# real-stanford/garmentnets

Hardware: AMD Instinct MI355X
Metric: garments/s end-to-end predict (PointNet++ -> gridding -> UNet3D -> WNF decode -> marching cubes) (higher is better)
Workload: dtype f32 (f16x2 convs, f16x2 decoder MLPs, fp32 accumulation)

## Files before the change

garmentnets_amd/_lib.py:

```python
import ctypes
import os

_HERE = os.path.dirname(os.path.abspath(__file__))
LIB_PATH = os.environ.get("GARMENTNETS_HIP_LIB") or os.path.join(_HERE, "libgarmentnets_hip.so")

GN_OK, GN_EINVAL, GN_ELAUNCH, GN_ECAP = 0, -1, -2, -3

_vp, _i32, _i64, _f32, _f64, _sz = (ctypes.c_void_p, ctypes.c_int, ctypes.c_int64, ctypes.c_float, ctypes.c_double,
                                   ctypes.c_size_t)

PROTOTYPES = {
    "gn_version": [],
    "gn_device_info": [_vp, _vp],
    "gn_segment_ptr": [_vp, _i64, _i32, _vp, _vp],
    "gn_fps": [_vp, _vp, _vp, _vp, _i32, _i32, _vp, _vp],
    "gn_fps_nested": [_vp, _vp, _vp, _vp, _i32, _i32, _vp, _vp, _vp, _vp],
    "gn_fps_workspace_bytes": [_i32, _i32],
    "gn_fps_nested_ws": [_vp, _vp, _vp, _vp, _i32, _i32, _vp, _vp, _vp, _vp, _sz, _vp],
    "gn_ball_query": [_vp, _vp, _vp, _vp, _i32, _i32, _f32, _i32, _vp, _vp, _vp],
    "gn_sa_gather": [_vp, _i32, _i32, _vp, _vp, _vp, _i32, _i32, _i32, _vp, _i32, _vp, _vp],
    "gn_segment_max": [_vp, _i32, _vp, _i32, _i32, _i32, _vp, _i32, _vp],
    "gn_sa_fused_supported": [_i32, _i32, _i32, _i32],
    "gn_sa_fused": [_vp, _i32, _i32, _vp, _vp, _vp, _vp, _i32, _i32, _i32, _vp, _vp, _vp, _vp, _i32, _i32, _i32, _vp, _i32, _vp],
    "gn_sa_fused_scoped": [_vp, _i32, _i32, _vp, _vp, _vp, _vp, _i32, _i32, _i32, _vp, _vp, _vp, _vp, _vp, _i32, _i32, _i32, _vp, _i32, _vp],
    "gn_sa_fused_group": [_vp, _i32, _i32, _vp, _vp, _vp, _vp, _i32, _i32, _i32, _vp, _vp, _vp, _vp, _vp, _i32, _i32, _i32, _vp, _i32, _vp, _i32],
    "gn_sa_fused_auto_group": [_i32, _i32, _i32, _i32, _i32],
    "gn_sa_gather_scoped": [_vp, _i32, _i32, _vp, _vp, _vp, _i32, _i32, _i32, _vp, _vp, _i32, _vp, _vp],
    "gn_global_max_pool": [_vp, _i32, _vp, _i32, _i32, _vp, _i32, _vp],
    "gn_knn_interpolate": [_vp, _i32, _vp, _vp, _vp, _vp, _i32, _i32, _i32, _i32, _vp, _i32, _vp],
    "gn_knn_interpolate_any": [_vp, _i32, _vp, _vp, _vp, _vp, _i32, _i32, _i32, _i32, _vp, _i32, _vp],
    "gn_linear": [_vp, _i32, _vp, _i32, _vp, _vp, _vp, _i32, _i64, _i32, _i32, _vp, _i32, _vp],
    "gn_nocs_head": [_vp, _i32, _i64, _i32, _vp, _vp, _vp, _vp],
    "gn_grid_features": [_vp, _i32, _i32, _vp, _vp, _vp, _vp, _i64, _vp, _vp, _vp, _i32, _i32, _vp, _i32, _vp, _vp],
    "gn_grid_scatter_workspace_bytes": [_i64, _i32, _i32],
    "gn_grid_scatter": [_vp, _i32, _vp, _i64, _i32, _i64, _i32, _vp, _vp, _vp, _sz, _i32, _vp],
    "gn_grid_scatter_ex": [_vp, _i32, _vp, _i64, _i32, _i32, _i64, _i32, _vp, _vp, _vp, _sz, _i32, _vp],
    "gn_channel_stats": [_vp, _i32, _i64, _i32, _vp, _vp, _vp],
    "gn_groupnorm_affine": [_vp, _vp, _i32, _i64, _vp, _vp, _i32, _i64, _i32, _i32, _i32, _f32, _vp, _vp, _vp, _vp, _vp, _vp],
    "gn_channel_stats_any": [_vp, _i32, _i64, _i32, _vp, _vp, _vp],
    "gn_groupnorm_affine_map": [_vp, _vp, _i32, _i32, _i64, _vp, _vp, _i32, _i32, _i64, _i32, _i32, _i32, _f32, _vp, _vp, _vp, _vp, _vp, _vp],
    "gn_conv3d_gcr": [_vp, _i32, _vp, _i32, _vp, _vp, _vp, _i32, _i32, _i32, _i32, _i32, _i32, _vp, _vp, _vp, _vp],
    "gn_conv3d_gcr_split": [_vp, _i32, _vp, _i32, _vp, _vp, _vp, _i32, _vp, _vp, _i32, _i32, _i32, _i32, _i32, _i32, _vp, _vp, _vp, _vp, _vp, _i32, _vp, _vp, _sz, _vp],
    "gn_conv3d_occupancy_workspace_bytes": [_i32, _i32, _i32, _i32],
    "gn_conv_affine_pack_bytes": [_i32, _i32, _i32],
    "gn_conv_affine_pack": [_vp, _i32, _i32, _vp, _vp, _vp, _vp, _i64, _vp, _i32, _vp, _sz, _vp, _vp, _vp, _vp, _vp, _sz, _vp],
    "gn_conv3d_gcr_split_persample": [_vp, _i32, _vp, _vp, _vp, _vp, _vp, _i32, _i32, _i32, _i32, _i32, _i32, _vp, _vp, _vp, _vp, _vp, _i32, _vp, _vp, _sz, _vp],
    "gn_conv_affine_pack_wino_bytes": [_i32, _i32, _i32],
    "gn_conv_affine_pack_wino": [_vp, _i32, _i32, _vp, _vp, _vp, _vp, _i64, _vp, _i32, _vp, _sz, _vp, _vp, _vp, _vp, _vp, _sz, _vp],
    "gn_conv3d_gcr_split_wino": [_vp, _i32, _vp, _vp, _vp, _vp, _vp, _vp, _i32, _i32, _i32, _i32, _i32, _i32, _vp, _vp, _vp, _vp, _vp, _i32, _vp, _sz, _vp],
    "gn_conv3d_gcr_split_wino_partial": [_vp, _i32, _vp, _vp, _vp, _vp, _vp, _vp, _i32, _i32, _i32, _i32, _i32, _i32, _vp, _vp, _vp, _vp, _vp],
    "gn_weight_pack_split_bytes": [_i32, _i32, _i32],
    "gn_weight_pack_split_wino_bytes": [_i32, _i32],
    "gn_weight_pack_upconv_bytes": [_i32, _i32],
    "gn_weight_pack_split": [_vp, _i32, _i32, _i32, _i32, _i32, _vp, _sz, _vp, _vp],
    "gn_weight_pack_split_wino": [_vp, _i32, _i32, _i32, _i32, _vp, _sz, _vp, _vp],
    "gn_weight_pack_upconv": [_vp, _i32, _i32, _i32, _i32, _vp, _sz, _vp, _vp],
    "gn_affine_act": [_vp, _i32, _i64, _i32, _vp, _vp, _vp, _i32, _vp, _vp],
    "gn_upconv_partial": [_vp, _i32, _vp, _vp, _vp, _i32, _vp, _vp, _i32, _i32, _i32, _i32, _i32, _vp, _vp],
    "gn_grid_tile_flags": [_vp, _i64, _i32, _i32, _i32, _i32, _i32, _vp, _vp],
    "gn_maxpool3d_2": [_vp, _i32, _i32, _i32, _i32, _i32, _vp, _vp, _vp, _vp],
    "gn_grid_stats": [_vp, _vp, _i64, _i32, _i64, _i32, _vp, _vp, _vp, _vp],
    "gn_trilinear_sample": [_vp, _i32, _i32, _i32, _i32, _vp, _i32, _i64, _i64, _vp, _i32, _vp],
    "gn_trilinear_sample_batch": [_vp, _i32, _i64, _i32, _i32, _i32, _i32, _vp, _i64, _vp, _i32, _vp],
    "gn_implicit_decode": [_vp, _i32, _i32, _i32, _i32, _vp, _i32, _vp, _i32, _i64, _i64, _vp, _vp, _vp, _vp, _i32, _vp, _vp, _vp, _vp, _i32,
                           _vp, _vp, _vp, _vp, _i32, _vp, _i32, _vp, _vp],
    "gn_ggm3d": [_vp, _i32, _i32, _i32, _f64, _vp, _vp, _vp],
    "gn_minmax": [_vp, _i64, _vp, _vp],
    "gn_ggm3d_batch": [_vp, _i32, _i32, _i32, _i32, _f64, _vp, _vp, _vp],
    "gn_ggm3d_range_workspace_bytes": [_i32, _i32, _i32, _i32],
    "gn_ggm3d_batch_ex": [_vp, _i32, _i32, _i32, _i32, _f64, _vp, _vp, _i32, _vp, _vp, _sz, _vp],
    "gn_minmax_batch": [_vp, _i32, _i64, _vp, _vp],
    "gn_mc33_batch_workspace_bytes": [_i32, _i32, _i32, _i32],
    "gn_mc33_batch": [_vp, _i32, _i32, _i32, _i32, _f64, _vp, _sz, _vp, _vp, _vp, _vp, _i64, _i64, _vp, _vp],
    "gn_mc33_batch_profiled": [_vp, _i32, _i32, _i32, _i32, _f64, _vp, _sz, _vp, _vp, _vp, _vp, _i64, _i64, _vp, _vp, _vp],
    "gn_mc33_workspace_bytes": [_i32, _i32, _i32],
    "gn_mc33": [_vp, _i32, _i32, _i32, _f64, _vp, _sz, _vp, _vp, _vp, _vp, _i64, _i64, _vp, _vp],
    "gn_gather_nn": [_vp, _i32, _i32, _i32, _vp, _i64, _f64, _vp, _vp],
    "gn_gather_nn_batch": [_vp, _i32, _i32, _i32, _i32, _vp, _i64, _f64, _vp, _vp],
    "gn_mesh_compact_workspace_bytes": [_i64, _i64],
    "gn_mesh_largest_component_workspace_bytes": [_i64],
    "gn_mesh_largest_component": [_vp, _i64, _i64, _vp, _sz, _vp, _vp, _vp, _vp],
    "gn_mesh_compact": [_vp, _i32, _vp, _vp, _i64, _i64, _vp, _sz, _vp, _vp, _vp, _vp],
    "gn_scale_verts": [_vp, _i64, _f64, _vp, _vp],
    "gn_implicit_decode_split": [_vp, _i32, _i64, _vp, _vp, _vp, _i32, _i32, _i32, _i32, _vp, _i32, _vp],
    "gn_implicit_decode_split_batch": [_vp, _i32, _i64, _i32, _vp, _vp, _vp, _i32, _i32, _i32, _i32, _vp, _i32, _vp],
    "gn_implicit_decode_batch": [_vp, _i32, _i64, _i32, _i32, _vp, _vp, _vp, _vp, _i32, _vp, _vp, _vp, _vp, _i32, _vp, _vp, _vp, _vp, _i32, _vp, _i32, _vp, _i32, _vp],
    "gn_implicit_decode_lattice_split": [_vp, _i32, _i32, _i32, _i32, _i32, _i64, _i64, _vp, _vp, _vp, _i32, _i32, _i32, _vp, _i32, _vp],
    "gn_decoder_input_scale": [_vp, _i64, _i32, _i32, _f32, _vp, _vp],
    "gn_nearest_neighbor": [_vp, _i64, _vp, _i64, _vp, _vp, _vp],
    "gn_nearest_neighbor_f64_batch": [_vp, _vp, _vp, _i32, _i64, _vp, _vp, _vp],
    "gn_point_mesh_sqdist_batch": [_vp, _vp, _vp, _vp, _i32, _i64, _vp, _vp, _vp, _vp],
    "gn_winding_number_batch": [_vp, _vp, _vp, _vp, _i32, _i64, _vp, _vp, _vp],
    "gn_winding_field_batch": [_vp, _vp, _vp, _i32, _i32, _i32, _i32, _vp, _vp, _vp],
    "gn_distance_field_batch": [_vp, _vp, _vp, _i32, _i32, _i32, _i32, _vp, _vp, _vp, _vp],
    "gn_query_targets_face_chunk": [],
    "gn_query_targets_workspace_bytes": [_i32, _i64, _i64, _i32],
    "gn_query_targets_batch": [_vp, _vp, _vp, _vp, _i32, _i64, _i64, _i32, _i32, _f32, _i32, _vp, _sz, _vp, _vp, _vp, _vp, _vp, _vp],
    "gn_nocs_bin_metrics_workspace_bytes": [_vp, _i32],
    "gn_nocs_bin_metrics": [_vp, _i32, _i32, _i32, _vp, _sz, _vp, _vp],
    "gn_value_losses_workspace_bytes": [_vp, _i32],
    "gn_value_losses": [_vp, _i32, _vp, _sz, _vp, _vp],
    "gn_nocs_bin_loss_bwd": [_vp, _i32, _i32, _i32, _vp, _vp, _vp, _vp],
    "gn_value_losses_bwd": [_vp, _i32, _vp, _vp, _vp],
    "gn_adam_step": [_vp, _i32, _i64, _vp, _i32, _vp],
    "gn_grad_pack": [_vp, _i32, _i64, _vp, _i64, _i32, _vp],
    "gn_grid_scatter_bwd_workspace_bytes": [_i64, _i32, _i64, _i32],
    "gn_grid_scatter_bwd": [_vp, _vp, _vp, _i32, _vp, _i64, _i32, _i32, _i64, _i32, _vp, _sz, _vp, _i32, _vp],
    "gn_segment_max_bwd": [_vp, _i32, _vp, _i32, _vp, _i32, _vp, _i32, _i32, _i32, _vp, _i32, _vp],
    "gn_global_max_pool_bwd": [_vp, _i32, _vp, _i32, _vp, _i32, _vp, _i32, _i32, _vp, _i32, _vp],
    "gn_sa_gather_bwd_workspace_bytes": [_i64, _i64],
    "gn_sa_gather_bwd": [_vp, _i32, _vp, _i64, _i32, _i64, _vp, _sz, _vp, _i32, _vp],
    "gn_knn_neighbours": [_vp, _vp, _vp, _vp, _i32, _i32, _i32, _vp, _vp, _vp],
    "gn_knn_interpolate_bwd_workspace_bytes": [_i64, _i32, _i64],
    "gn_knn_interpolate_bwd": [_vp, _vp, _i32, _i32, _vp, _i32, _i32, _i32, _vp, _sz, _vp, _i32, _vp],
    "gn_trilinear_sample_bwd_workspace_bytes": [_i32, _i64, _i32, _i32, _i32],
    "gn_trilinear_sample_bwd": [_vp, _i32, _vp, _i32, _i32, _i32, _i32, _i32, _vp, _i64, _vp, _sz, _vp, _vp, _vp],
    "gn_conv3d_bwd_weight_workspace_bytes": [_i32, _i32, _i32, _i32, _i32, _i32],
    "gn_conv3d_bwd_weight": [_vp, _i32, _vp, _i32, _vp, _vp, _vp, _vp, _i32, _i32, _i32, _i32, _i32, _vp, _sz, _vp, _vp],
    "gn_relu_mask": [_vp, _vp, _i64, _vp, _vp],
    "gn_relu_mask_max_workspace_bytes": [_i32],
    "gn_relu_mask_max": [_vp, _vp, _i32, _i64, _i32, _vp, _vp, _vp, _vp, _vp, _sz, _vp],
    "gn_conv3d_bwd_weight_split_workspace_bytes": [_i32, _i32, _i32, _i32, _i32, _i32],
    "gn_conv3d_bwd_weight_split": [_vp, _i32, _vp, _i32, _vp, _vp, _vp, _vp, _vp, _vp, _i32, _i32, _i32, _i32, _i32, _vp, _sz, _vp, _vp],
    "gn_groupnorm_bwd_stats_workspace_bytes": [_i32, _i64, _i32],
    "gn_groupnorm_bwd_stats": [_vp, _i32, _i32, _vp, _i32, _i32, _i32, _i32, _i32, _i32, _vp, _sz, _vp, _vp, _vp],
    "gn_groupnorm_bwd_coef": [_vp, _vp, _vp, _vp, _i32, _i32, _i64, _vp, _vp, _vp, _vp, _i32, _i32, _i64, _i32, _i32, _i32, _f32, _vp, _vp, _vp, _vp, _vp,
                              _vp, _vp],
    "gn_groupnorm_bwd_apply": [_vp, _i32, _i32, _vp, _i32, _i32, _i32, _i32, _i32, _i32, _vp, _vp, _vp, _i32, _i32, _i32, _vp, _vp],
    "gn_maxpool3d_2_bwd": [_vp, _vp, _i32, _i32, _i32, _i32, _i32, _vp, _vp],
    "gn_linear_act_bwd_workspace_bytes": [_i64, _i32],
    "gn_linear_act_bwd": [_vp, _i32, _vp, _i32, _vp, _i64, _i32, _vp, _i32, _vp, _sz, _vp, _vp],
    "gn_linear_bwd_weight_workspace_bytes": [_i64, _i32, _i32],
    "gn_linear_bwd_weight": [_vp, _i32, _vp, _i32, _i64, _i32, _i32, _vp, _sz, _vp, _i32, _vp],
    "gn_row_affine": [_vp, _i32, _vp, _vp, _i64, _i32, _vp, _i32, _vp],
    "gn_col_moments_workspace_bytes": [_i64, _i32],
    "gn_col_moments": [_vp, _i32, _i64, _i32, _vp, _sz, _vp, _vp],
    "gn_col_dots_workspace_bytes": [_i64, _i32],
    "gn_col_dots": [_vp, _i32, _vp, _i32, _i64, _i32, _vp, _sz, _vp, _vp],
    "gn_bn_train_bwd_workspace_bytes": [_i64, _i32],
    "gn_bn_train_bwd": [_vp, _i32, _vp, _i32, _vp, _i64, _i32, _vp, _i32, _vp, _sz, _vp, _vp],
    "gn_resident_points": [_vp, _vp, _i32, _i32, _vp, _vp, _vp, _vp, _vp, _vp, _vp, _vp],
    "gn_resident_garment": [_vp, _vp, _i32, _i32, _vp, _vp, _vp, _vp, _vp, _vp, _vp, _vp, _vp, _vp],
    "gn_resident_volume": [_vp, _vp, _i32, _i32, _i32, _vp, _vp, _vp, _vp, _vp, _i32, _vp, _vp, _vp],
    "gn_resident_volume_queries": [_vp, _vp, _i32, _i32, _i32, _vp, _vp, _vp, _vp, _vp, _vp, _vp, _vp],
    "gn_resident_query_targets": [_vp, _vp, _i32, _i64, _i32, _i64, _i64, _i32, _i32, _f32, _i32, _vp, _vp, _sz, _vp, _vp, _vp],
    "gn_resident_surface": [_vp, _vp, _i32, _i32, _vp, _vp, _i32, _vp, _vp, _vp, _vp],
    "gn_resident_mc_surface": [_vp, _vp, _i32, _i32, _vp, _vp, _vp, _vp, _vp],
    "gn_render_points_batch": [_vp, _vp, _vp, _vp, _vp, _i32, _i32, _vp, _vp],
    "gn_color_idx_batch": [_vp, _vp, _vp, _vp, _vp, _i32, _i32, _vp, _vp],
}
_RESTYPES = {"gn_weight_pack_split_bytes": _sz, "gn_weight_pack_split_wino_bytes": _sz, "gn_weight_pack_upconv_bytes": _sz,
             "gn_conv_affine_pack_bytes": _sz, "gn_conv_affine_pack_wino_bytes": _sz, "gn_conv3d_occupancy_workspace_bytes": _sz, "gn_mc33_workspace_bytes": _sz, "gn_ggm3d_range_workspace_bytes": _sz, "gn_mc33_batch_workspace_bytes": _sz, "gn_grid_scatter_workspace_bytes": _sz, "gn_fps_workspace_bytes": _sz, "gn_mesh_compact_workspace_bytes": _sz, "gn_mesh_largest_component_workspace_bytes": _sz,
             "gn_nocs_bin_metrics_workspace_bytes": _sz, "gn_value_losses_workspace_bytes": _sz,
             "gn_grid_scatter_bwd_workspace_bytes": _sz, "gn_sa_gather_bwd_workspace_bytes": _sz, "gn_knn_interpolate_bwd_workspace_bytes": _sz,
             "gn_trilinear_sample_bwd_workspace_bytes": _sz, "gn_conv3d_bwd_weight_workspace_bytes": _sz, "gn_conv3d_bwd_weight_split_workspace_bytes": _sz, "gn_relu_mask_max_workspace_bytes": _sz, "gn_groupnorm_bwd_stats_workspace_bytes": _sz,
             "gn_linear_act_bwd_workspace_bytes": _sz, "gn_linear_bwd_weight_workspace_bytes": _sz,
             "gn_col_moments_workspace_bytes": _sz, "gn_col_dots_workspace_bytes": _sz, "gn_bn_train_bwd_workspace_bytes": _sz,
             "gn_query_targets_workspace_bytes": _sz}

LINEAR_BWD_CHUNK_ROWS = 512
LINEAR_ACT_CHUNK_ROWS = 1024

LOSS_MAX_SETS = 8
LOSS_KINDS = {"l2": 0, "smooth_l1": 1, "bce_logits": 2, "row_norm": 3}


class NocsBinSet(ctypes.Structure):
    _fields_ = [("logits", _vp), ("gt", _vp), ("n", _i64), ("ldl", _i32), ("pad", _i32)]


class LossSegment(ctypes.Structure):
    _fields_ = [("pred", _vp), ("target", _vp), ("count", _i64), ("kind", _i32), ("mirror", _i32)]


class NocsBinGradSet(ctypes.Structure):
    _fields_ = [("logits", _vp), ("gt", _vp), ("grad", _vp), ("n", _i64), ("ldl", _i32), ("ldg", _i32), ("ncols", _i32), ("pad", _i32)]


class LossGradSegment(ctypes.Structure):
    _fields_ = [("pred", _vp), ("target", _vp), ("grad", _vp), ("count", _i64), ("coef", _f64), ("kind", _i32), ("mirror", _i32)]


QT_KINDS = {"nocs_winding_number_field": 0, "sim_nocs_winding_number_field": 0, "nocs_distance_field": 1, "nocs_signed_distance_field": 2,
            "nocs_occupancy_grid": 3}

ADAM_CHUNK = 4096
ADAM_MAX_HYPER = 16


class AdamEntry(ctypes.Structure):
    _fields_ = [("p", _vp), ("g", _vp), ("exp_avg", _vp), ("exp_avg_sq", _vp), ("numel", _i64), ("blk0", _i64), ("hyper", _i32), ("pad", _i32)]


class PackEntry(ctypes.Structure):
    _fields_ = [("src", _vp), ("dst_off", _i64), ("numel", _i64), ("blk0", _i64)]


class AdamHyper(ctypes.Structure):
    _fields_ = [("lr", _f64), ("beta1", _f64), ("beta2", _f64), ("eps", _f64), ("weight_decay", _f64), ("bias_correction1", _f64),
                ("bias_correction2_sqrt", _f64)]


RESIDENT_META = ("pc_off", "pc_len", "vert_off", "face_off", "num_faces", "mc_vert_off", "mc_face_off", "num_mc_faces", "dataset_idx",
# ... 62 lines not shown
```

garmentnets_amd/arith.py:

```python
import dataclasses
import os

CONV_FP32, SPLIT_BF16X2, SPLIT_BF16X3, SPLIT_F16X2 = 0, 2, 3, 4
CONV_MODE_NAMES = {"fp32": CONV_FP32, "f16x2": SPLIT_F16X2, "bf16x3": SPLIT_BF16X3, "bf16x2": SPLIT_BF16X2}
DECODE_MODES = ("f16x2", "fp32")
CONV_GRAD_MODES = ("fp32", "f16x2")


def _env_choice(name, default, choices):
    v = os.environ.get(name, default)
    if v not in choices:
        raise ValueError(f"{name}={v!r}: expected one of {sorted(choices)}")
    return v


def _env_flag(name, default=True):
    return os.environ.get(name, "1" if default else "0") != "0"


@dataclasses.dataclass(frozen=True)
class Arith:
    conv_mode: int = SPLIT_F16X2
    decode_mode: str = "f16x2"
    sparse_first_conv: bool = True
    affine_in_weights: bool = True
    winograd: bool = True
    winograd32: bool = True
    polyphase_upconv: bool = True
    fold_final_conv: bool = True
    fused_lattice: bool = True
    ggm_fp32: bool = False
    device_packs: bool = False
    conv_grad_mode: str = "fp32"

    def __post_init__(self):
        if self.conv_mode not in CONV_MODE_NAMES.values():
            raise ValueError(f"conv_mode={self.conv_mode!r}")
        if self.decode_mode not in DECODE_MODES:
            raise ValueError(f"decode_mode={self.decode_mode!r}")
        if self.conv_grad_mode not in CONV_GRAD_MODES:
            raise ValueError(f"conv_grad_mode={self.conv_grad_mode!r}: expected one of {list(CONV_GRAD_MODES)}")
        if self.conv_mode == SPLIT_BF16X2:
            import warnings
            warnings.warn("garmentnets_amd: conv_mode bf16x2 is a PREVIEW arithmetic -- it does not guarantee the 1e-4 WNF tolerance (0.9-1.2e-4 "
                          "observed on the G=32 goldens) and a finite over-tolerance result is not caught by predict's NaN fallback; use f16x2 "
                          "(default), bf16x3 or fp32 for results held to the reference's tolerance", RuntimeWarning, stacklevel=3)

    @classmethod
    def named(cls, conv="f16x2", decode="f16x2", **kw):
        return cls(conv_mode=CONV_MODE_NAMES[conv], decode_mode=decode, **kw)

    @classmethod
    def from_env(cls):
        return cls(conv_mode=CONV_MODE_NAMES[_env_choice("GARMENTNETS_CONV_MODE", "f16x2", CONV_MODE_NAMES)],
                   decode_mode=_env_choice("GARMENTNETS_DECODE_MODE", "f16x2", DECODE_MODES),
                   sparse_first_conv=_env_flag("GARMENTNETS_SPARSE_CONV"), affine_in_weights=_env_flag("GARMENTNETS_AFFINE_IN_WEIGHTS"),
                   winograd=_env_flag("GARMENTNETS_WINOGRAD"), winograd32=_env_flag("GARMENTNETS_WINOGRAD32"), polyphase_upconv=_env_flag("GARMENTNETS_POLYPHASE"),
                   fold_final_conv=_env_flag("GARMENTNETS_FOLD_FINAL_CONV"), fused_lattice=_env_flag("GARMENTNETS_FUSED_LATTICE"),
                   ggm_fp32=_env_flag("GARMENTNETS_GGM_FP32", False), device_packs=_env_flag("GARMENTNETS_DEVICE_PACKS", False),
                   conv_grad_mode=_env_choice("GARMENTNETS_CONV_GRAD_MODE", "fp32", CONV_GRAD_MODES))

    def replace(self, **kw):
        return dataclasses.replace(self, **kw)

    @property
    def split(self):
        return self.conv_mode != CONV_FP32 or self.decode_mode != "fp32"

    def strict_fp32(self):
        return self.replace(conv_mode=CONV_FP32, decode_mode="fp32", conv_grad_mode="fp32")

    @property
    def conv_name(self):
        return {v: k for k, v in CONV_MODE_NAMES.items()}[self.conv_mode]


DEFAULT = Arith.from_env()
```

garmentnets_amd/components/unet3d.py:

```python
import functools
from typing import NamedTuple, Optional

import torch
from torch import nn

from .. import arith as AR
from .. import ops
from .mlp import PackedModule, pack_wb, param_cache


def number_of_features_per_level(init_channel_number, num_levels):
    return [init_channel_number * 2 ** k for k in range(num_levels)]


CHANNEL_GRANULE = 32


def stored_channels(c):
    return -(-int(c) // CHANNEL_GRANULE) * CHANNEL_GRANULE


class _Layout(tuple):
    real = property(lambda self: self[0])
    stored = property(lambda self: self[1])
    cout = property(lambda self: self[2])


def to_stored(v, real, stored):
    if tuple(real) == tuple(stored):
        return v
    out = v.new_zeros(tuple(v.shape[:-1]) + (sum(stored),))
    o = k = 0
    for r, st in zip(real, stored):
        out[..., o:o + r] = v[..., k:k + r]
        o, k = o + st, k + r
    return out


class AtRest(NamedTuple):
    flat: Optional[torch.Tensor]
    reach: int
    value: Optional[torch.Tensor] = None
    small: Optional[torch.Tensor] = None


class ConvPlan(NamedTuple):
    mode: int
    aiw: bool
    wino: bool
    poly: bool
    small: int


@functools.lru_cache(maxsize=None)
def conv_plan(arith, dims, c0, c1, cout, reach=0, rest_known=False, small=None, cells=False, rest0=False):
    mode, (D, H, W) = arith.conv_mode, dims
    if mode == ops.CONV_FP32:
        return ConvPlan(mode, False, False, False, 0)
    poly = c1 > 0 and arith.polyphase_upconv and mode != ops.SPLIT_BF16X3 and c1 <= 384
    wino = (c1 == 0 or (poly and cout % 128 != 0)) and arith.winograd and mode == ops.SPLIT_F16X2 and ops.wino_supported(c0, cout, dims)
    if wino and cout % 128 == 0:
        wino = (D // 4) * (H // 8) * (W // 8) * (cout // 128) >= 32
    elif wino:
        wino = arith.winograd32 and (D // 8) * (H // 8) * (W // 8) * (cout // 32) >= 512
    aiw = arith.affine_in_weights and mode == ops.SPLIT_F16X2 and c0 % 16 == 0 and cout % 32 == 0
    aiw = aiw and ((c1 == 0 and (reach == 1 or (reach > 1 and rest_known))) or (poly and rest0))
    occ = (cells and reach > 0 and arith.sparse_first_conv and c1 == 0 and mode != ops.SPLIT_BF16X3 and c0 <= 384 and (cout % 128 == 0 or cout % 64 != 0)
           and min(dims) > 2 * reach and (reach == 1 or small is not None)
           and (not wino or small is None or ops.wino_supported(c0, cout, small)))
    return ConvPlan(mode, bool(aiw), bool(wino), bool(poly), (int(small[0]) if small is not None else 8 if wino else 5) if occ else 0)


class ConvGradPlan(NamedTuple):
    data: str
    weight: str


def grad_data_pack_unsupported(cout_stored):
    return cout_stored % 16 != 0


def grad_weight_partial_quad(c0, c1):
    return c0 % 4 != 0 or c1 % 4 != 0


@functools.lru_cache(maxsize=None)
def conv_grad_plan(arith, dims, c0, c1, cout_stored):
    if arith.conv_grad_mode != "f16x2":
        return ConvGradPlan("fp32", "fp32")
    return ConvGradPlan("fp32" if grad_data_pack_unsupported(cout_stored) else "f16x2", "fp32" if grad_weight_partial_quad(c0, c1) else "f16x2")


_ACT = {"r": ("ReLU", lambda: nn.ReLU(inplace=True), ops.ACT_RELU), "l": ("LeakyReLU", lambda: nn.LeakyReLU(negative_slope=0.1, inplace=True), ops.ACT_LEAKY),
        "e": ("ELU", lambda: nn.ELU(inplace=True), ops.ACT_ELU)}


def _class_constants(small_out, reach, cout):
    B, n = small_out.shape[0], small_out.shape[1]
    pos = [0, n // 2, n - 1] if reach == 1 else [0, 1, n // 2, n - 2, n - 1]
    k = small_out
    for dim in (1, 2, 3):
        k = torch.cat([k.narrow(dim, q, 1) for q in pos], dim=dim)
    return k.reshape(B, len(pos) ** 3, cout).contiguous()


class SingleConv(PackedModule, nn.Sequential):

    def __init__(self, in_channels, out_channels, kernel_size=3, order="gcr", num_groups=8, padding=1):
        super().__init__()
        if kernel_size != 3 or padding != 1:
            raise NotImplementedError("garmentnets_amd implements the 3x3x3, padding 1 SingleConv of the GarmentNets pipeline")
        if "c" not in order or order.count("c") != 1:
            raise ValueError("Conv layer MUST be present (exactly once)")
        if order[0] in "rle":
            raise ValueError("Non-linearity cannot be the first operation in the layer")
        if any(ch not in "bgrlec" for ch in order):
            raise ValueError(f"Unsupported layer type in {order!r}. MUST be one of ['b', 'g', 'r', 'l', 'e', 'c']")
        if any(ch in "rle" for ch in order[:order.index("c")]) or sum(ch in "gb" for ch in order[:order.index("c")]) > 1:
            raise NotImplementedError(f"layer order {order!r}: at most one normalisation and no non-linearity in front of the convolution")
        self.order = order
        self.in_real = None
        for i, ch in enumerate(order):
            before = i < order.index("c")
            nch = in_channels if before else out_channels
            if ch in _ACT:
                self.add_module(_ACT[ch][0], _ACT[ch][1]())
            elif ch == "c":
                self.add_module("conv", nn.Conv3d(in_channels, out_channels, 3, padding=1, bias=not ("g" in order or "b" in order)))
            elif ch == "g":
                groups = num_groups if nch >= num_groups else 1
                assert nch % groups == 0, f"Expected number of channels in input to be divisible by num_groups. num_channels={nch}, num_groups={groups}"
                self.add_module("groupnorm", nn.GroupNorm(num_groups=groups, num_channels=nch))
            elif ch == "b":
                self.add_module("batchnorm", nn.BatchNorm3d(nch))

    def _pack(self):
        wp = ops.pack_conv_weight(self.conv.weight) if self.conv.in_channels % 16 == 0 else None
        gn = getattr(self, "groupnorm", None)
        return wp, (None if gn is None else gn.weight.detach().float().contiguous()), (None if gn is None else gn.bias.detach().float().contiguous())

    def _layout(self, src0, src1):
        stored = (src0.shape[-1],) if src1 is None else (src0.shape[-1], src1.shape[-1])
        real = stored if self.in_real is None else tuple(self.in_real)
        cout = self.conv.out_channels
        if self.in_real is not None and (len(real) != len(stored) or any(r > st for r, st in zip(real, stored))):
            raise ValueError(f"SingleConv: inputs of {stored} stored channels for {real} real ones")
        if real == stored and cout % CHANNEL_GRANULE == 0:
            return None
        return _Layout((real, stored, stored_channels(cout)))

    def _padded_weight(self, lay):
        def build():
            w = self.conv.weight.detach()
            wp = w.new_zeros((lay.cout, sum(lay.stored)) + tuple(w.shape[2:]))
            wp[:w.shape[0]] = to_stored(w.transpose(1, -1), lay.real, lay.stored).transpose(1, -1)
            return wp.contiguous()
        return param_cache(self, "_split_packs").get(self._gen(lay), "padded_weight", build)

    def _gen(self, lay):
        w = self.conv.weight
        return (w.device, w._version) if lay is None else (w.device, w._version, lay)

    def _norm_affine(self, ch, B, st0, st1, real=None, stored=None):
        if ch == "g":
            return ops.groupnorm_affine(st0, st1, self.groupnorm.num_groups, self.groupnorm.eps, self.groupnorm.weight.detach().float().contiguous(),
                                        self.groupnorm.bias.detach().float().contiguous(), real=real)
        bn = self.batchnorm
        sc = (bn.weight.detach().double() / torch.sqrt(bn.running_var.double() + bn.eps))
        sh = bn.bias.detach().double() - bn.running_mean.double() * sc
        if real is not None:
            sc, sh = to_stored(sc, real, stored), to_stored(sh, real, stored)
        return sc.float().expand(B, -1).contiguous(), sh.float().expand(B, -1).contiguous()

    def _run_generic(self, src0, src1, stats0, stats1, with_stats, lay=None):
        order, ic = self.order, self.order.index("c")
        B, cout = src0.shape[0], self.conv.out_channels if lay is None else lay.cout
        cin = src0.shape[-1] + (0 if src1 is None else src1.shape[-1])
        if lay is None:
            wp, _, _ = self.packed()
        else:
            wp = param_cache(self, "_split_packs").get(self._gen(lay), "fp32", lambda: ops.pack_conv_weight(self._padded_weight(lay)))
        if ic == 0:
            a = torch.ones((B, cin), dtype=torch.float32, device=src0.device)
            d = torch.zeros_like(a)
        else:
            st0 = st1 = None
            if order[0] == "g":
                st0 = stats0 if stats0 is not None else ops.channel_stats(src0)
                st1 = None if src1 is None else (stats1 if stats1 is not None else ops.channel_stats(src1))
            a, d = self._norm_affine(order[0], B, st0, st1, *((None, None) if lay is None else (lay.real, lay.stored)))
        post = order[ic + 1:]
        bias = None if self.conv.bias is None else self.conv.bias.detach().float().contiguous()
        if bias is not None and lay is not None:
            bias = to_stored(bias, (self.conv.out_channels,), (cout,)).contiguous()
        out_lay = (None, None) if lay is None else ((self.conv.out_channels,), (cout,))
        fuse_relu = bias is None and post[:1] == "r"
        y = ops.conv3d_gcr(src0, src1, a, d, wp, cout, relu=fuse_relu)
        k = 1 if fuse_relu else 0
        if bias is not None:
            act = _ACT[post[0]][2] if post[:1] and post[0] in _ACT else ops.ACT_NONE
            ops.affine_act(y, bias=bias, act=act, out=y)
            k = 1 if act != ops.ACT_NONE else 0
        for ch in post[k:]:
            if ch in _ACT:
                ops.affine_act(y, act=_ACT[ch][2], out=y)
            else:
                na, nd = self._norm_affine(ch, B, ops.channel_stats(y) if ch == "g" else None, None, *out_lay)
                ops.affine_act(y, a=na, d=nd, out=y)
        return y, (ops.channel_stats(y) if with_stats else None)

    def run(self, src0, src1=None, stats0=None, stats1=None, with_stats=True, arith=None, rest0=None):
        return self._run(src0, src1, stats0, stats1, with_stats, arith, None, rest0)[:2]

    def run_at_rest(self, src0, at_rest, stats0=None, with_stats=True, arith=None):
        return self._run(src0, None, stats0, None, with_stats, arith, at_rest, None)

    def _run(self, src0, src1, stats0, stats1, with_stats, arith, at_rest, rest0):
        arith = arith or AR.DEFAULT
        lay = self._layout(src0, src1)
        if self.order != "gcr":
            return self._run_generic(src0, src1, stats0, stats1, with_stats, lay) + (None,)
        wp, gamma, beta = self.packed()
        st0 = stats0 if stats0 is not None else ops.channel_stats(src0)
        st1 = None
        if src1 is not None:
            st1 = stats1 if stats1 is not None else ops.channel_stats(src1)
        cout = self.conv.out_channels if lay is None else lay.cout
        reach, value, small, flat = (0, None, None, None) if at_rest is None else (at_rest.reach, at_rest.value, at_rest.small, at_rest.flat)
        plan = conv_plan(arith, tuple(src0.shape[1:4]), src0.shape[-1], 0 if src1 is None else src1.shape[-1], cout, reach, value is not None,
                         None if small is None else tuple(small.shape[1:4]), flat is not None, rest0 is not None)
        if plan.mode == ops.CONV_FP32:
            a, d = ops.groupnorm_affine(st0, st1, self.groupnorm.num_groups, self.groupnorm.eps, gamma, beta, real=None if lay is None else lay.real)
            if lay is not None:
                wp = param_cache(self, "_split_packs").get(self._gen(lay), "fp32", lambda: ops.pack_conv_weight(self._padded_weight(lay)))
            r, nxt = ops.conv3d_gcr(src0, src1, a, d, wp, cout, relu=True, with_stats=with_stats), None
        else:
            r, nxt = self._run_split(plan, src0, src1, st0, st1, with_stats, at_rest, gamma, beta, rest0, lay, device_packs=arith.device_packs)
        return (r + (nxt,)) if with_stats else (r, None, nxt)

    def _run_split(self, plan, src0, src1, st0, st1, with_stats, at_rest, gamma, beta, rest0, lay=None, device_packs=False):
        gn, weight, cout, mode, c0 = self.groupnorm, self.conv.weight, self.conv.out_channels, plan.mode, src0.shape[-1]
        real = None
        if lay is not None:
            weight, cout, real = self._padded_weight(lay), lay.cout, lay.real
        cache, gen = param_cache(self, "_split_packs"), self._gen(lay)
        device_packs = bool(device_packs) and weight.is_cuda

        def raw():
            w = weight.detach()
            return w if w.dtype == torch.float32 and w.is_contiguous() else w.float().contiguous()
        part = prep = act_inv = rest_out = None
        if plan.aiw and not plan.poly:
            a, d = ops.groupnorm_affine(st0, None, gn.num_groups, gn.eps, gamma, beta, real=real)
            prep = ops.conv_affine_pack(weight if weight.is_contiguous() else weight.contiguous(), a, d, st0, at_rest.value if at_rest.reach > 1 else None,
                                        wino=plan.wino)
            rest_out = torch.relu(prep.kbias[:, 63]).contiguous()
        else:
            if mode == ops.SPLIT_F16X2:
                a, d, act_inv = ops.groupnorm_affine(st0, st1, gn.num_groups, gn.eps, gamma, beta, with_act_scale=True, real=real)
            else:
                a, d = ops.groupnorm_affine(st0, st1, gn.num_groups, gn.eps, gamma, beta, real=real)
            if plan.poly:
                def build_poly():
                    w0, wm, _ = ops.polyphase_weights(weight, c0)
                    return (ops.pack_conv_weight_split(w0, mode).to(weight.device), ops.pack_upconv_weight(wm, cout, mode).to(weight.device))
                if device_packs:
                    pk0, pkm = cache.get(gen, ("device", "poly", mode, c0), lambda: (ops.pack_conv_weight_split_device(raw(), mode, 0, c0),
                                                                                     ops.pack_upconv_weight_device(raw(), c0, mode)))
                else:
                    pk0, pkm = cache.get(gen, ("poly", mode, c0), build_poly)
                part = ops.upconv_partial(src1, a[:, c0:].contiguous(), d[:, c0:].contiguous(), pkm, cout, act_inv=act_inv)
                if plan.aiw:
                    a0 = (a[:, :c0] * act_inv[:, None]).contiguous()
                    d0 = (d[:, :c0] * act_inv[:, None]).contiguous()
                    w0c = cache.get(gen, ("w0", c0), lambda: weight.detach()[:, :c0].contiguous())
                    prep = ops.conv_affine_pack(w0c, a0, d0, st0, rest0, wino=plan.wino)
                else:
                    a, d = a[:, :c0].contiguous(), d[:, :c0].contiguous()
                    if not plan.wino:
                        pack = pk0
                    elif device_packs:
                        pack = cache.get(gen, ("device", "poly_wino", c0), lambda: ops.pack_conv_weight_split_wino_device(raw(), 0, c0))
                    else:
                        pack = cache.get(gen, ("poly_wino", c0), lambda: ops.pack_conv_weight_split_wino(ops.polyphase_weights(weight, c0)[0]).to(weight.device))
            elif plan.wino and device_packs:
                pack = cache.get(gen, ("device", "wino"), lambda: ops.pack_conv_weight_split_wino_device(raw()))
            elif plan.wino:
                pack = cache.get(gen, "wino", lambda: ops.pack_conv_weight_split_wino(weight).to(weight.device))
            elif device_packs:
                pack = cache.get(gen, ("device", mode), lambda: ops.pack_conv_weight_split_device(raw(), mode))
            else:
                pack = cache.get(gen, mode, lambda: ops.pack_conv_weight_split(weight, mode).to(weight.device))
        if prep is not None:
            launch = lambda x, **kw: ops.conv3d_gcr_split_persample(x, prep, relu=True, **kw)
        elif plan.wino:
            launch = lambda x, **kw: ops.conv3d_gcr_split_wino(x, a, d, pack, cout, relu=True, act_inv=act_inv, **kw)
        else:
            launch = lambda x, **kw: ops.conv3d_gcr_split(x, None if plan.poly else src1, a, d, pack, cout, relu=True, act_inv=act_inv, **kw)
        occ, small_out = {}, None
        if plan.small:
            B, n, reach = src0.shape[0], plan.small, at_rest.reach
            small_out = launch(at_rest.small if at_rest.small is not None else torch.zeros((B, n, n, n, c0), dtype=torch.float32, device=src0.device))
            occ = dict(tile_active=ops.grid_tile_flags(at_rest.flat, B, src0.shape[1:4], reach), kconst=_class_constants(small_out, reach, cout), kreach=reach)
        r = launch(src0, with_stats=with_stats, partial=part, **occ)
        learned = rest_out is not None or small_out is not None
        return r, (AtRest(at_rest.flat, at_rest.reach + 1, rest_out, small_out) if learned else None)


class DoubleConv(nn.Sequential):
    def __init__(self, in_channels, out_channels, encoder, kernel_size=3, order="gcr", num_groups=8):
        super().__init__()
        if encoder:
            c1_in, c1_out = in_channels, max(out_channels // 2, in_channels)
            c2_in, c2_out = c1_out, out_channels
        else:
            c1_in, c1_out = in_channels, out_channels
            c2_in, c2_out = out_channels, out_channels
        self.add_module("SingleConv1", SingleConv(c1_in, c1_out, kernel_size, order, num_groups))
        self.add_module("SingleConv2", SingleConv(c2_in, c2_out, kernel_size, order, num_groups))
        if encoder:
            self.SingleConv1.in_real = (c1_in,)
        self.SingleConv2.in_real = (c2_in,)

    def run(self, src0, src1=None, stats0=None, stats1=None, sparse_flat=None, arith=None, rest0=None):
        if sparse_flat is None or src1 is not None:
            y, st = self.SingleConv1.run(src0, src1, stats0, stats1, arith=arith, rest0=rest0)
            return self.SingleConv2.run(y, None, st, arith=arith) + (None,)
        y, st, at_rest = self.SingleConv1.run_at_rest(src0, AtRest(sparse_flat, 1), stats0, arith=arith)
        y, st, at_rest = self.SingleConv2.run_at_rest(y, at_rest, st, arith=arith)
        return y, st, (None if at_rest is None else at_rest.value)


class Encoder(nn.Module):
    def __init__(self, in_channels, out_channels, apply_pooling=True, conv_layer_order="gcr", num_groups=8):
        super().__init__()
        self.pooling = nn.MaxPool3d(kernel_size=2) if apply_pooling else None
        self.basic_module = DoubleConv(in_channels, out_channels, encoder=True, order=conv_layer_order, num_groups=num_groups)

    def run(self, x, stats=None, sparse_flat=None, arith=None):
        if self.pooling is not None:
            sparse_flat = None
            x, stats = ops.maxpool3d_2(x, with_stats=True)
        return self.basic_module.run(x, None, stats, sparse_flat=sparse_flat, arith=arith)


class Decoder(nn.Module):
    def __init__(self, in_channels, out_channels, conv_layer_order="gcr", num_groups=8):
        super().__init__()
        self.basic_module = DoubleConv(in_channels, out_channels, encoder=False, order=conv_layer_order, num_groups=num_groups)
        self.basic_module.SingleConv1.in_real = (out_channels, in_channels - out_channels)

    def run(self, encoder_features, x, stats_skip=None, stats_x=None, arith=None, skip_rest=None):
        return self.basic_module.run(encoder_features, x, stats_skip, stats_x, arith=arith, rest0=skip_rest)[:2]


class FinalConv1x1(PackedModule, nn.Conv3d):
    in_stored = None

    def stored_weight(self):
        w = self.weight.detach().reshape(self.out_channels, self.in_channels)
        return to_stored(w, (self.in_channels,), (self.in_stored or self.in_channels,))

    def _pack(self):
        return pack_wb(self.stored_weight(), self.bias)

    def run(self, x):
        wp, b, k = self.packed()
        shp = x.shape
        if shp[-1] != k:
            raise ValueError(f"FinalConv1x1: input of {shp[-1]} channels, expected {k}")
        y = ops.linear(x.reshape(-1, shp[-1]), wp, b, None, None, relu=False, K=k)
        return y.reshape(*shp[:-1], self.out_channels)


class Abstract3DUNet(nn.Module):
    def __init__(self, in_channels, out_channels, final_sigmoid=False, basic_module=DoubleConv, f_maps=64, layer_order="gcr",
                 num_groups=8, num_levels=4, is_segmentation=False, testing=False, **kwargs):
        super().__init__()
        if basic_module is not DoubleConv or is_segmentation:
            raise NotImplementedError("only the DoubleConv regression UNet of the GarmentNets pipeline is implemented")
        if isinstance(f_maps, int):
            f_maps = number_of_features_per_level(f_maps, num_levels=num_levels)
        self.f_maps = list(f_maps)
        self.encoders = nn.ModuleList([
            Encoder(in_channels if i == 0 else f_maps[i - 1], f, apply_pooling=i > 0, conv_layer_order=layer_order, num_groups=num_groups)
            for i, f in enumerate(f_maps)])
        rf = list(reversed(f_maps))
        self.decoders = nn.ModuleList([
            Decoder(rf[i] + rf[i + 1], rf[i + 1], conv_layer_order=layer_order, num_groups=num_groups) for i in range(len(rf) - 1)])
        self.final_conv = FinalConv1x1(f_maps[0], out_channels, 1)
        self.final_conv.in_stored = stored_channels(f_maps[0])
        self.final_activation = None
        self.in_channels = in_channels
        self.arith = None

    def check_input(self, x):
        if x.shape[-1] % 16 != 0:
            raise NotImplementedError(f"Abstract3DUNet.run: an input stored with {x.shape[-1]} channels is not a multiple of 16 (the first convolution "
                                      "reads 16 channels at a time): hand it channel-padded (stored_channels), as forward() and the volume aggregator do")
        k = 2 ** (len(self.encoders) - 1)
        if any(int(n) % k != 0 for n in x.shape[1:4]):
            raise NotImplementedError(f"Abstract3DUNet: grid {tuple(x.shape[1:4])} does not halve evenly through {len(self.encoders)} levels "
                                      f"(every dimension must be a multiple of {k}: only x2 nearest upsampling is implemented)")

    def run(self, x, stats=None, pre_final=False, return_stats=False, sparse_flat=None, arith=None):
        self.check_input(x)
        feats = []
        for i, enc in enumerate(self.encoders):
            x, stats, rest_out = enc.run(x, stats, sparse_flat=sparse_flat if i == 0 else None, arith=arith)
            feats.insert(0, (x, stats, rest_out))
        for dec, (skip, skip_stats, skip_rest) in zip(self.decoders, feats[1:]):
            x, stats = dec.run(skip, x, skip_stats, stats, arith=arith, skip_rest=skip_rest)
        if pre_final:
            return (x, stats) if return_stats else x
        return self.final_conv.run(x)

    def forward(self, x):
        return self.run(*stored_input(x), arith=self.arith).permute(0, 4, 1, 2, 3)


def stored_input(x):
    stats = getattr(x, "_gn_stats", None)
    v = stored_volume(x)
    if v.shape[-1] % 16 != 0:
        v, stats = to_stored(v, (v.shape[-1],), (stored_channels(v.shape[-1]),)), None
    return v, stats


def stored_volume(x):
    v = getattr(x, "_gn_stored", None)
    return to_channel_last(x) if v is None else v


def to_channel_last(x):
    return x.permute(0, 2, 3, 4, 1).contiguous()
```

garmentnets_amd/csrc/split_conv.h:

```cpp
#pragma once
#include "common.h"

#define SP_KS 16

__device__ __forceinline__ int sp_axis_class(int z, int D, int r) { return z < r ? z : (z >= D - r ? 2 * r - (D - 1 - z) : r); }
__device__ __forceinline__ int sp_axis_mask(int g, int n) { return (g > 0 ? 1 : 0) | (g < n - 1 ? 2 : 0); }

struct SplitArgs {
    const float *src0;
    const float *src1;
    const float *a;
    const float *d;
    const uint4 *wp;
    float *out;
    double *osum;
    double *osq;
    int C0, C1, B, D, H, W, Cout, relu;
    int tiles_y, tiles_x;
    const float *out_scale;
    const float *act_inv;
    const int *active_list;
    const int *active_count;
    const float *kconst;
    const float *partial;
    const float *kbias;
    int64_t wp_bstride;
    int osc_bstride;
    int kreach;
    int chain;
};

__device__ __forceinline__ bool sp_work_item(const SplitArgs &p, int ncb, int tiles_per_sample, int &b, int &tile, int &cb) {
    unsigned nblk = gridDim.x, lin = blockIdx.x;
    if (p.active_list) {
        nblk = (unsigned)(*p.active_count) * (unsigned)ncb;
        lin = blockIdx.y * gridDim.x + blockIdx.x;
        if (lin >= nblk) return false;
    }
    const unsigned xcd = lin & 7u, jx = lin >> 3, qx = nblk >> 3, rx = nblk & 7u;
    const unsigned logical = (xcd < rx ? xcd * (qx + 1) : rx * (qx + 1) + (xcd - rx) * qx) + jx;
    const unsigned t = logical / (unsigned)ncb;
    cb = (int)(logical % (unsigned)ncb);
    if (p.active_list) {
        const int item = p.active_list[t];
        b = item / tiles_per_sample;
        tile = item - b * tiles_per_sample;
    } else {
        b = blockIdx.y;
        tile = (int)t;
    }
    return true;
}

template <int P, int HZ = GN_CONV_HZ> struct HaloLayout {
    static constexpr int VB = P * 32;
    static constexpr int ROWP = GN_CONV_HX * VB + 16;
    static constexpr int BYTES = HZ * GN_CONV_HY * ROWP;
    __device__ static constexpr __forceinline__ int at(int hz, int hy, int hx) { return (hz * GN_CONV_HY + hy) * ROWP + hx * VB; }
};

void gn_launch_conv3d_wino(const SplitArgs &p, int tiles, hipStream_t st);
void gn_launch_conv3d_wino32(const SplitArgs &p, int tiles8, hipStream_t st);
```

garmentnets_amd/csrc/unet_split.hip:

```cpp
#include "common.h"
#include "split_conv.h"

__device__ __forceinline__ void sp_store_frag_full(const SplitArgs &p, const f32x16 &val, float osc, float *ob, const float *pb, double &ssum, double &ssq,
                                                   const float *kb = nullptr, bool interior = true, int gz = 0, int gy = 0, int gx = 0) {
    const int64_t rs = (int64_t)p.W * p.Cout;
    float pv[16];
    float kv[16];
    if (kb) {
        if (interior) {
            const float k63 = kb[63 * (int64_t)p.Cout];
#pragma unroll
            for (int q = 0; q < 16; ++q) kv[q] = k63;
        } else {
            const int mz = sp_axis_mask(gz, p.D);
#pragma unroll
            for (int q = 0; q < 16; ++q) kv[q] = kb[(int64_t)((mz * 4 + sp_axis_mask(gy + (q >> 2), p.H)) * 4 + sp_axis_mask(gx + (q & 3), p.W)) * p.Cout];
        }
    }
    if (pb) {
        const int64_t prs = (int64_t)(p.W >> 1) * 8 * p.Cout;
#pragma unroll
        for (int q = 0; q < 16; ++q) {
            const int j = q >> 2, k = q & 3;
            pv[q] = pb[(j >> 1) * prs + (int64_t)((k >> 1) * 8 + (j & 1) * 2 + (k & 1)) * p.Cout];
// ... 685 lines not shown
    for (int u = 0; u < NT; ++u) { ssum[u] = 0.0; ssq[u] = 0.0; }
    const bool full = z0 + TZ <= p.D && y0 + GN_CONV_TY <= p.H && x0 + GN_CONV_TX <= p.W;
    const bool interior = z0 > 0 && z0 + TZ < p.D && y0 > 0 && y0 + GN_CONV_TY < p.H && x0 > 0 && x0 + GN_CONV_TX < p.W;
#pragma unroll
    for (int t = 0; t < 2; ++t)
#pragma unroll
        for (int u = 0; u < NT; ++u) {
            const int n = n0 + u * 32 + r;
            const float osn = p.out_scale[(int64_t)b * p.osc_bstride + n];
            const float osc = p.act_inv ? __fmul_rn(osn, p.act_inv[b]) : osn;
            const float *kb = p.kbias ? p.kbias + (int64_t)b * 64 * p.Cout + n : nullptr;
            if (full) {
                const int gy = y0 + t * 4, gx = x0 + 4 * h;
                float *ob = p.out + ((((int64_t)b * p.D + gz) * p.H + gy) * p.W + gx) * p.Cout + n;
                const float *pb = p.partial ? p.partial + ((((int64_t)b * (p.D >> 1) + (gz >> 1)) * (p.H >> 1) + (gy >> 1)) * (p.W >> 1) + (gx >> 1)) * (8 * p.Cout) + ((gz & 1) * 4 * p.Cout + n) : nullptr;
                sp_store_frag_full(p, tot[t][u], osc, ob, pb, ssum[u], ssq[u], kb, interior, gz, gy, gx);
                continue;
            }
#pragma unroll
            for (int q = 0; q < 16; ++q) {
                const int i = (q & 3) + 8 * (q >> 2) + 4 * h;
                const int gy = y0 + t * 4 + (i >> 3), gx = x0 + (i & 7);
                if (gz < p.D && gy < p.H && gx < p.W) {
                    float v;
                    v = __fmul_rn(tot[t][u][q], osc);
                    if (kb) v = __fadd_rn(v, kb[(int64_t)((sp_axis_mask(gz, p.D) * 4 + sp_axis_mask(gy, p.H)) * 4 + sp_axis_mask(gx, p.W)) * p.Cout]);
                    if (p.partial) v = __fadd_rn(v, p.partial[((((int64_t)b * (p.D >> 1) + (gz >> 1)) * (p.H >> 1) + (gy >> 1)) * (p.W >> 1) + (gx >> 1)) * (8 * p.Cout) + (((gz & 1) * 4 + (gy & 1) * 2 + (gx & 1)) * p.Cout + n)]);
                    if (p.relu) v = gn_relu(v);
                    p.out[((((int64_t)b * p.D + gz) * p.H + gy) * p.W + gx) * p.Cout + n] = v;
                    ssum[u] += (double)v;
                    ssq[u] += (double)v * (double)v;
                }
            }
        }
    if (p.osum) {
        double *red = reinterpret_cast<double *>(smem);
#pragma unroll
        for (int u = 0; u < NT; ++u) {
            const double s2 = ssum[u] + __shfl_xor(ssum[u], 32), q2 = ssq[u] + __shfl_xor(ssq[u], 32);
            if (h == 0) { red[(cg * 4 + zs) * 64 + u * 32 + r] = s2; red[512 + (cg * 4 + zs) * 64 + u * 32 + r] = q2; }
        }
        __syncthreads();
        if (tid < 128) {
            const int g = tid >> 6, c = tid & 63;
            const double *rs = red + g * 256 + c, *rq = red + 512 + g * 256 + c;
            const double s4 = rs[0] + rs[64] + rs[128] + rs[192];
            const double q4 = rq[0] + rq[64] + rq[128] + rq[192];
            atomicAdd(&p.osum[(int64_t)b * p.Cout + cb * 128 + tid], s4);
            atomicAdd(&p.osq[(int64_t)b * p.Cout + cb * 128 + tid], q4);
        }
    }
}


__global__ __launch_bounds__(1024) void occ_compact_kernel(const unsigned char *__restrict__ flags, int B, int tz4, int tyx, int pair,
                                                           int *__restrict__ list, int *__restrict__ count) {
    const int Tz = pair == 2 ? (tz4 + 1) / 2 : tz4, Tk = tyx * Tz, total = B * Tk;
    __shared__ int wsum[16];
    __shared__ int running;
    const int tid = threadIdx.x, lane = tid & 63, wave = tid >> 6;
    if (tid == 0) running = 0;
    __syncthreads();
    for (int base = 0; base < total; base += 1024) {
        const int i = base + tid;
        bool act = false;
        if (i < total) {
            const int b = i / Tk, t = i - b * Tk, yx = t / Tz, z = t - yx * Tz;
            const unsigned char *f = flags + ((int64_t)b * tyx + yx) * tz4;
            act = pair == 2 ? (f[2 * z] != 0 || (2 * z + 1 < tz4 && f[2 * z + 1] != 0)) : f[z] != 0;
        }
        const unsigned long long m = __ballot(act);
        const int before = __popcll(m & ((1ull << lane) - 1ull));
        if (lane == 0) wsum[wave] = __popcll(m);
        __syncthreads();
        int off = running;
        for (int w = 0; w < wave; ++w) off += wsum[w];
        if (act) list[off + before] = i;
        __syncthreads();
        if (tid == 0) {
            int tsum = 0;
            for (int w = 0; w < 16; ++w) tsum += wsum[w];
            running += tsum;
        }
        __syncthreads();
    }
    if (tid == 0) *count = running;
}

__global__ __launch_bounds__(256) void conv_fill_inactive_kernel(SplitArgs p, const unsigned char *__restrict__ flags, int pair) {
    const int TZ = GN_CONV_TZ * pair, tz4 = (p.D + GN_CONV_TZ - 1) / GN_CONV_TZ, tiles_z = (p.D + TZ - 1) / TZ;
    const int tx = blockIdx.x % p.tiles_x, ty = blockIdx.x / p.tiles_x, b = blockIdx.y;
    const unsigned char *fl = flags + ((int64_t)b * p.tiles_y * p.tiles_x + (int64_t)ty * p.tiles_x + tx) * tz4;
    const int y0 = ty * GN_CONV_TY, x0 = tx * GN_CONV_TX, r = p.kreach, nc = 2 * r + 1;
    const int quads = p.Cout >> 2, tid = threadIdx.x;
    const int vpp = 256 / quads, quad = tid % quads, vl = tid / quads;
    const bool yx_inner = y0 >= r && y0 + GN_CONV_TY <= p.H - r && x0 >= r && x0 + GN_CONV_TX <= p.W - r;
    const float *kc = p.kconst + (int64_t)b * (nc * nc * nc) * p.Cout + quad * 4;
    const float4 centre = *reinterpret_cast<const float4 *>(kc + (int64_t)((r * nc + r) * nc + r) * p.Cout);
    double s4[4] = {0.0, 0.0, 0.0, 0.0}, q4[4] = {0.0, 0.0, 0.0, 0.0};
    if (vl < vpp) {
        for (int tz = 0; tz < tiles_z; ++tz) {
            if (fl[pair * tz] || (pair == 2 && pair * tz + 1 < tz4 && fl[pair * tz + 1])) continue;
            const int z0 = tz * TZ;
            const bool uniform = yx_inner && z0 >= r && z0 + TZ <= p.D - r;
            float *ob = p.out + ((((int64_t)b * p.D + z0) * p.H + y0) * p.W + x0) * p.Cout + quad * 4;
            if (uniform) {
                int cnt = 0;
                for (int v = vl; v < TZ * 64; v += vpp, ++cnt)
                    *reinterpret_cast<float4 *>(ob + (((int64_t)(v >> 6) * p.H + ((v >> 3) & 7)) * p.W + (v & 7)) * p.Cout) = centre;
                const double n = (double)cnt;
                s4[0] += n * (double)centre.x; s4[1] += n * (double)centre.y; s4[2] += n * (double)centre.z; s4[3] += n * (double)centre.w;
                q4[0] += n * ((double)centre.x * (double)centre.x); q4[1] += n * ((double)centre.y * (double)centre.y);
                q4[2] += n * ((double)centre.z * (double)centre.z); q4[3] += n * ((double)centre.w * (double)centre.w);
                continue;
            }
            for (int v = vl; v < TZ * 64; v += vpp) {
                const int gz = z0 + (v >> 6), gy = y0 + ((v >> 3) & 7), gx = x0 + (v & 7);
                if (gz >= p.D || gy >= p.H || gx >= p.W) continue;
                const int cls = (sp_axis_class(gz, p.D, r) * nc + sp_axis_class(gy, p.H, r)) * nc + sp_axis_class(gx, p.W, r);
                const float4 cv = *reinterpret_cast<const float4 *>(kc + (int64_t)cls * p.Cout);
                *reinterpret_cast<float4 *>(p.out + ((((int64_t)b * p.D + gz) * p.H + gy) * p.W + gx) * p.Cout + quad * 4) = cv;
                s4[0] += (double)cv.x; s4[1] += (double)cv.y; s4[2] += (double)cv.z; s4[3] += (double)cv.w;
                q4[0] += (double)cv.x * (double)cv.x; q4[1] += (double)cv.y * (double)cv.y; q4[2] += (double)cv.z * (double)cv.z; q4[3] += (double)cv.w * (double)cv.w;
            }
        }
    }
    if (!p.osum) return;
    __shared__ double red[256][8];
#pragma unroll
    for (int i = 0; i < 4; ++i) { red[tid][i] = s4[i]; red[tid][4 + i] = q4[i]; }
    __syncthreads();
    if (vl == 0) {
#pragma unroll
        for (int i = 0; i < 4; ++i) {
            double a = 0.0, c = 0.0;
            for (int k = 0; k < vpp; ++k) { a += red[tid + k * quads][i]; c += red[tid + k * quads][4 + i]; }
            if (a != 0.0 || c != 0.0) {
                atomicAdd(&p.osum[(int64_t)b * p.Cout + quad * 4 + i], a);
                atomicAdd(&p.osq[(int64_t)b * p.Cout + quad * 4 + i], c);
            }
        }
    }
}

extern "C" size_t gn_conv3d_occupancy_workspace_bytes(int B, int D, int H, int W) {
    if (B < 0 || D <= 0 || H <= 0 || W <= 0) return 0;
    return ((size_t)B * gn_cdiv(D, GN_CONV_TZ) * gn_cdiv(H, GN_CONV_TY) * gn_cdiv(W, GN_CONV_TX) + 16) * sizeof(int);
}

static int conv3d_gcr_split_impl(const float *src0, int C0, const float *src1, int C1, const float *a, const float *d,
                                 const void *wp_planes, int mode, const float *out_scale, const float *act_inv_scale, int B, int D, int H,
                                 int W, int Cout, int relu, float *out, double *out_sum, double *out_sumsq, const unsigned char *tile_active,
                                 const float *kconst, int kreach, const float *partial, const float *kbias, int64_t wp_bstride, int osc_bstride,
                                 void *occ_ws, size_t occ_ws_bytes, void *stream, int wino = 0) {
    GN_REQUIRE(B >= 0 && D > 0 && H > 0 && W > 0 && C0 > 0 && C1 >= 0 && Cout > 0, "gn_conv3d_gcr_split: bad sizes");
    GN_REQUIRE(mode == GN_SPLIT_BF16X2 || mode == GN_SPLIT_BF16X3 || mode == GN_SPLIT_F16X2, "gn_conv3d_gcr_split: mode must be GN_SPLIT_BF16X2, _BF16X3 or _F16X2");
    GN_REQUIRE(out_scale != nullptr, "gn_conv3d_gcr_split: out_scale [Cout] is required (ones for the bf16 modes)");
    GN_REQUIRE(C0 % SP_KS == 0 && C1 % SP_KS == 0 && Cout % 32 == 0, "gn_conv3d_gcr_split: channel counts must be multiples of 16 (in) / 32 (out)");
    GN_REQUIRE(C1 == 0 || (src1 && D % 2 == 0 && H % 2 == 0 && W % 2 == 0), "gn_conv3d_gcr_split: upsampled source needs even dims");
    GN_REQUIRE((out_sum == nullptr) == (out_sumsq == nullptr), "gn_conv3d_gcr_split: out_sum and out_sumsq must come together");
    if (B == 0) return GN_OK;
    hipStream_t st = gn_stream(stream);
    if (out_sum) {
        GN_HIP(gn_zero_stats(out_sum, out_sumsq, (size_t)B * Cout, st), "gn_conv3d_gcr_split");
    }
    SplitArgs p;
    p.src0 = src0; p.src1 = src1; p.a = a; p.d = d; p.wp = (const uint4 *)wp_planes; p.out = out; p.osum = out_sum; p.osq = out_sumsq;
    p.C0 = C0; p.C1 = C1; p.B = B; p.D = D; p.H = H; p.W = W; p.Cout = Cout; p.relu = relu; p.out_scale = out_scale; p.act_inv = act_inv_scale;
    p.active_list = nullptr; p.active_count = nullptr; p.kconst = kconst; p.kreach = kreach; p.partial = partial;
    p.kbias = kbias; p.wp_bstride = wp_bstride; p.osc_bstride = osc_bstride; p.chain = 1;
    GN_REQUIRE(!partial || (D % 2 == 0 && H % 2 == 0 && W % 2 == 0), "gn_conv3d_gcr_split: a polyphase partial needs even dims");
    const int tz = (int)gn_cdiv(D, GN_CONV_TZ);
    p.tiles_y = (int)gn_cdiv(H, GN_CONV_TY);
    p.tiles_x = (int)gn_cdiv(W, GN_CONV_TX);
    const int tiles = tz * p.tiles_y * p.tiles_x;
    const int Cin_total = C0 + C1;
    const bool fits32 = (int64_t)D * H * W * C0 * 4 < ((int64_t)1 << 32);
    const bool wide128 = !wino && mode != GN_SPLIT_BF16X3 && Cout % 128 == 0 && Cin_total <= 384 && fits32 && (int64_t)tiles * (Cout / 128) * B >= 512;
    const bool wino32 = wino && Cout % 128 != 0;
    GN_REQUIRE(!wino || wino32 || (mode == GN_SPLIT_F16X2 && C1 == 0 && !partial && Cout % 128 == 0 && C0 <= 256 && fits32 && D % GN_CONV_TZ == 0 && H % GN_CONV_TY == 0 &&
                                   W % GN_CONV_TX == 0 && (int64_t)D * H * W <= ((int64_t)1 << 27)),
               "gn_conv3d_gcr_split_wino: needs one source, Cin <= 256, Cout %% 128 == 0, D %% 4 == H %% 8 == W %% 8 == 0, D*H*W <= 2^27 and "
               "D*H*W*Cin*4 < 2^32");
    GN_REQUIRE(!wino32 || (mode == GN_SPLIT_F16X2 && C1 == 0 && C0 <= 128 && fits32 && D % 8 == 0 && H % 8 == 0 && W % 8 == 0 && (int64_t)D * H * W <= ((int64_t)1 << 27)),
               "gn_conv3d_gcr_split_wino (Cout %% 128 != 0): needs one source, Cin <= 128, D %% 8 == H %% 8 == W %% 8 == 0, D*H*W <= 2^27 and D*H*W*Cin*4 < 2^32");
    const int tiles8 = (int)gn_cdiv(D, 8) * p.tiles_y * p.tiles_x;
    const bool strip = !wino && mode != GN_SPLIT_BF16X3 && !wide128 && C1 == 0 && (int64_t)tiles8 * (Cout / 32) * B >= 512;
    const bool wide = !wino && !wide128 && !strip && (Cout % 64 == 0) && ((int64_t)tiles * (Cout / 64) * B >= 1024);
#define SP_LAUNCH(P_, F16_)                                                                                                    \
    do {                                                                                                                       \
        if (wide) hipLaunchKernelGGL((conv3d_split_kernel<2, P_, F16_>), dim3(tiles * (Cout / 64), B), dim3(256), 0, st, p);    \
        else hipLaunchKernelGGL((conv3d_split_kernel<1, P_, F16_>), dim3(tiles * (Cout / 32), B), dim3(256), 0, st, p);        \
        gn_note_kernel(wide ? "conv3d_split_kernel<2, " #P_ ", " #F16_ ">" : "conv3d_split_kernel<1, " #P_ ", " #F16_ ">");     \
    } while (0)
    GN_REQUIRE((tile_active == nullptr) == (kconst == nullptr), "gn_conv3d_gcr_split: tile_active and kconst come together");
    GN_REQUIRE(!(tile_active && partial), "gn_conv3d_gcr_split: the occupancy-aware launch cannot take a polyphase partial (inactive tiles are "
                                          "filled with the border-class constants alone: the partial would be dropped there)");
    GN_REQUIRE(!tile_active || ((kreach == 1 || kreach == 2) && mode != GN_SPLIT_BF16X3 && D > 2 * kreach && H > 2 * kreach && W > 2 * kreach),
               "gn_conv3d_gcr_split: the occupancy-aware launch needs a two-plane mode, kreach 1 or 2 and dims > 2 kreach");
    if (tile_active) {
        GN_REQUIRE(occ_ws && occ_ws_bytes >= gn_conv3d_occupancy_workspace_bytes(B, D, H, W) && ((uintptr_t)occ_ws & 3) == 0,
                   "gn_conv3d_gcr_split: the occupancy-aware launch needs gn_conv3d_occupancy_workspace_bytes(B, D, H, W) bytes of workspace");
        GN_REQUIRE(Cout % 4 == 0 && Cout <= 1024, "gn_conv3d_gcr_split: the occupancy-aware launch needs Cout <= 1024");
        const int pair = (strip || wino32) ? 2 : 1;
        int *count = (int *)occ_ws, *list = count + 16;
        hipLaunchKernelGGL(occ_compact_kernel, dim3(1), dim3(1024), 0, st, tile_active, B, tz, p.tiles_y * p.tiles_x, pair, list, count);
        hipLaunchKernelGGL(conv_fill_inactive_kernel, dim3(p.tiles_y * p.tiles_x, B), dim3(256), 0, st, p, tile_active, pair);
        p.active_list = list;
        p.active_count = count;
    }
    if (wino32) {
        gn_launch_conv3d_wino32(p, tiles8, st);
        gn_note_kernel("conv3d_split_wino32pc_kernel<true>");
    } else if (wino) {
        gn_launch_conv3d_wino(p, tiles, st);
        gn_note_kernel("conv3d_split_wino_kernel<true>");
    } else if (strip) {
        if (mode == GN_SPLIT_F16X2) hipLaunchKernelGGL((conv3d_split_strip_kernel<true>), dim3(tiles8 * (Cout / 32), B), dim3(256), 0, st, p);
        else hipLaunchKernelGGL((conv3d_split_strip_kernel<false>), dim3(tiles8 * (Cout / 32), B), dim3(256), 0, st, p);
        gn_note_kernel(mode == GN_SPLIT_F16X2 ? "conv3d_split_strip_kernel<true>" : "conv3d_split_strip_kernel<false>");
    } else if (wide128) {
        if (mode == GN_SPLIT_F16X2) hipLaunchKernelGGL((conv3d_split_wide_kernel<2, true>), dim3(tiles * (Cout / 128), B), dim3(512), 0, st, p);
        else hipLaunchKernelGGL((conv3d_split_wide_kernel<2, false>), dim3(tiles * (Cout / 128), B), dim3(512), 0, st, p);
        gn_note_kernel(mode == GN_SPLIT_F16X2 ? "conv3d_split_wide_kernel<2, true>" : "conv3d_split_wide_kernel<2, false>");
    } else
    if (mode == GN_SPLIT_BF16X3) SP_LAUNCH(3, false);
    else if (mode == GN_SPLIT_BF16X2) SP_LAUNCH(2, false);
    else SP_LAUNCH(2, true);
#undef SP_LAUNCH
    GN_LAUNCH_CHECK("gn_conv3d_gcr_split");
    return GN_OK;
}

extern "C" int gn_conv3d_gcr_split(const float *src0, int C0, const float *src1, int C1, const float *a, const float *d,
                                   const void *wp_planes, int mode, const float *out_scale, const float *act_inv_scale, int B, int D, int H,
                                   int W, int Cout, int relu, float *out, double *out_sum, double *out_sumsq, const unsigned char *tile_active,
                                   const float *kconst, int kreach, const float *partial, void *occ_ws, size_t occ_ws_bytes, void *stream) {
    return conv3d_gcr_split_impl(src0, C0, src1, C1, a, d, wp_planes, mode, out_scale, act_inv_scale, B, D, H, W, Cout, relu, out, out_sum, out_sumsq,
                                 tile_active, kconst, kreach, partial, nullptr, 0, 0, occ_ws, occ_ws_bytes, stream);
}

extern "C" int gn_conv3d_gcr_split_persample(const float *src, int Cin, const float *stage_a, const float *stage_d, const void *pack,
                                             const float *out_scale, const float *kbias, int B, int D, int H, int W, int Cout, int relu, float *out,
                                             double *out_sum, double *out_sumsq, const unsigned char *tile_active, const float *kconst, int kreach,
                                             const float *partial, void *occ_ws, size_t occ_ws_bytes, void *stream) {
    GN_REQUIRE(kbias != nullptr && pack != nullptr, "gn_conv3d_gcr_split_persample: pack and kbias are required");
    GN_REQUIRE(Cin > 0 && Cin % SP_KS == 0 && Cout > 0 && Cout % 32 == 0, "gn_conv3d_gcr_split_persample: channel counts must be multiples of 16 (in) / 32 (out)");
    const int64_t per_sample = (int64_t)(Cin / SP_KS) * 27 * (Cout / 32) * 2 * 1024;
    return conv3d_gcr_split_impl(src, Cin, nullptr, 0, stage_a, stage_d, pack, GN_SPLIT_F16X2, out_scale, nullptr, B, D, H, W, Cout, relu, out, out_sum,
                                 out_sumsq, tile_active, kconst, kreach, partial, kbias, per_sample, Cout, occ_ws, occ_ws_bytes, stream);
}

static int conv3d_wino_entry(const float *src, int Cin, const float *a, const float *d, const void *pack, const float *out_scale,
                             const float *act_inv_scale, const float *kbias, int B, int D, int H, int W, int Cout, int relu, float *out,
                             double *out_sum, double *out_sumsq, const unsigned char *tile_active, const float *kconst, int kreach,
                             const float *partial, void *occ_ws, size_t occ_ws_bytes, void *stream) {
    GN_REQUIRE(pack != nullptr && Cin > 0 && Cin % SP_KS == 0 && Cout > 0 && Cout % 32 == 0, "gn_conv3d_gcr_split_wino: pack, Cin %% 16 == 0 and Cout %% 32 == 0 are required");
    GN_REQUIRE(!(kbias && act_inv_scale), "gn_conv3d_gcr_split_wino: the affine-in-weights form carries its scales in out_scale [B][Cout]");
    GN_REQUIRE(!partial || Cout % 128 != 0, "gn_conv3d_gcr_split_wino32: a polyphase partial goes with the 32-wide column-block kernel (Cout %% 128 != 0)");
    const int64_t per_sample = kbias ? (int64_t)(Cin / SP_KS) * 36 * (Cout / 32) * 2 * 1024 : 0;
    return conv3d_gcr_split_impl(src, Cin, nullptr, 0, a, d, pack, GN_SPLIT_F16X2, out_scale, act_inv_scale, B, D, H, W, Cout, relu, out, out_sum,
                                 out_sumsq, tile_active, kconst, kreach, partial, kbias, per_sample, kbias ? Cout : 0, occ_ws, occ_ws_bytes, stream, 1);
}

extern "C" int gn_conv3d_gcr_split_wino(const float *src, int Cin, const float *a, const float *d, const void *pack, const float *out_scale,
                                        const float *act_inv_scale, const float *kbias, int B, int D, int H, int W, int Cout, int relu, float *out,
                                        double *out_sum, double *out_sumsq, const unsigned char *tile_active, const float *kconst, int kreach,
                                        void *occ_ws, size_t occ_ws_bytes, void *stream) {
    return conv3d_wino_entry(src, Cin, a, d, pack, out_scale, act_inv_scale, kbias, B, D, H, W, Cout, relu, out, out_sum, out_sumsq, tile_active, kconst,
                             kreach, nullptr, occ_ws, occ_ws_bytes, stream);
}

extern "C" int gn_conv3d_gcr_split_wino_partial(const float *src, int Cin, const float *a, const float *d, const void *pack, const float *out_scale,
                                                const float *act_inv_scale, const float *kbias, int B, int D, int H, int W, int Cout, int relu, float *out,
                                                double *out_sum, double *out_sumsq, const float *partial, void *stream) {
    GN_REQUIRE(partial != nullptr, "gn_conv3d_gcr_split_wino_partial: partial is required (gn_conv3d_gcr_split_wino is the entry without one)");
    return conv3d_wino_entry(src, Cin, a, d, pack, out_scale, act_inv_scale, kbias, B, D, H, W, Cout, relu, out, out_sum, out_sumsq, nullptr, nullptr,
                             1, partial, nullptr, 0, stream);
}
```

garmentnets_amd/csrc/unet_wino.hip:

```cpp
#include "split_conv.h"

struct WinoLayout {
    static constexpr int VB = 64;
    static constexpr int ROWP = 4 * VB + 16;
    static constexpr int HZ = GN_CONV_TZ + 2, HY = GN_CONV_TY + 2;
    static constexpr int SLOT = HZ * HY * ROWP;
    static constexpr int NSLOT = 5;
};

template <bool F16>
__global__ __launch_bounds__(512, 1) void conv3d_split_wino_kernel(SplitArgs p) {
    constexpr int P = 2, NT = 2;
    using WL = WinoLayout;
    constexpr int STEPB = 2 * NT * P * 1024;
    constexpr int GB = 3 * STEPB;
    constexpr int RING = 3;
    constexpr int HALO_BYTES = WL::NSLOT * WL::SLOT;
    constexpr int AD_OFF = HALO_BYTES + RING * GB;
    constexpr int ADN = 256;
    constexpr int NIT = 6;
    constexpr int ST_OFF = AD_OFF + 2 * ADN * 4;
    constexpr int EC_OFF = ST_OFF + 2 * 128 * 8;
    __shared__ __attribute__((aligned(16))) unsigned char smem[EC_OFF + 2 * 128 * 4];
    const unsigned lds_ring = (unsigned)(size_t)(__attribute__((address_space(3))) unsigned char *)smem + HALO_BYTES;
// ... 131 lines not shown
            _Pragma("unroll") for (int q = 0; q < 16; ++q) {                                                                   \
                const float m = AC[u][q];                                                                                      \
                if ((J) <= 2) tot[0][u][q] = __fadd_rn(tot[0][u][q], m);                                                       \
                if ((J) == 1) tot[1][u][q] = __fadd_rn(tot[1][u][q], m);                                                       \
                if ((J) >= 2) tot[1][u][q] = __fsub_rn(tot[1][u][q], m);                                                       \
            }                                                                                                                  \
    } while (0)

    bool fresh = true;
    int sbase = 0;
    for (;;) {
        if (fresh) {
            GN_WAIT_VM_LGKM0(0);
            __syncthreads();
            {
                int tf = threadIdx.x;
                asm volatile("" : "+v"(tf));
                if (tf < Cin) { adl[tf] = p.a[(int64_t)b * Cin + tf]; adl[ADN + tf] = p.d[(int64_t)b * Cin + tf]; }
                if (tf < 256) stl[tf] = 0.0;
                if (tf < 128) {
                    const float osn = p.out_scale[(int64_t)b * p.osc_bstride + cb * 128 + tf];
                    ecl[tf] = p.act_inv ? __fmul_rn(osn, p.act_inv[b]) : osn;
                    ecl[128 + tf] = p.kbias ? p.kbias[((int64_t)b * 64 + 63) * p.Cout + cb * 128 + tf] : 0.f;
                }
            }
            bgs = reinterpret_cast<const unsigned char *>(p.wp) + (int64_t)b * p.wp_bstride + (int64_t)cb * STEPB;
#pragma unroll
            for (int i = 0; i < 6; ++i) WN_ISSUE_PIECE(i / 3, i % 3);
            base0 = p.src0 + (int64_t)b * p.D * p.H * p.W * p.C0;
            set_rows(z0, y0, x0);
            issue_rows(0);
            GN_WAIT_VM_LGKM0(0);
            __syncthreads();
            affine_rows(0);
#pragma unroll
            for (int j = 0; j < 4; ++j) convert(j, j);
            __syncthreads();
            sbase = 0;
            WN_READ(0, 0, 0, 0);
            fresh = false;
        }
#pragma unroll
        for (int u = 0; u < NT; ++u)
#pragma unroll
            for (int q = 0; q < 16; ++q) { acc[u][q] = 0.f; tot[0][u][q] = 0.f; tot[1][u][q] = 0.f; }
        const int nitem = item + 32;
        const bool more = nitem < item_end;
        int bn = b, cbn = cb, z0n = z0, y0n = y0, x0n = x0;
        if (more) decode(nitem, bn, cbn, z0n, y0n, x0n);
        const bool cont = more && bn == b && cbn == cb;

        for (int s = 0; s < nslices; ++s) {
            const bool last = s + 1 == nslices;
            const int sn = last ? (cont ? 0 : s) : s + 1;
            if (last && cont) set_rows(z0n, y0n, x0n);
            const int64_t wrap = last && cont ? -(int64_t)nslices * 36 * bstep : 0;
            const int nbase = sbase == 0 ? 4 : sbase - 1;
            int slo[4], nslo[4];
#pragma unroll
            for (int j = 0; j < 4; ++j) {
                const int a_ = sbase + j, n_ = nbase + j;
                slo[j] = (a_ >= WL::NSLOT ? a_ - WL::NSLOT : a_) * WL::SLOT;
                nslo[j] = n_ >= WL::NSLOT ? n_ - WL::NSLOT : n_;
            }
#pragma unroll
            for (int g = 0; g < 12; ++g) {
                const int j = g / 3, dz = g % 3, X = g & 1, Y = X ^ 1;
                if (g == 1) GN_WAIT_VM_ONLY(2 + NIT);
                else if (g == 3 || g == 5 || g == 8 || g == 11) GN_WAIT_VM_LGKM0(2);
                else if (g > 0 || s > 0) GN_WAIT_VM_ONLY(2);
                if (g > 0 || s > 0) __builtin_amdgcn_s_barrier();
                WN_READ(Y, slo[j], dz * WL::HY + 1, (g % RING) * GB + STEPB);
                __builtin_amdgcn_sched_barrier(0);
                if (g == 10) bgs += wrap;
                if (g == 2 || g == 4 || g == 7 || g == 10) {
                    const int jn = g == 2 ? 0 : g == 4 ? 1 : g == 7 ? 2 : 3;
                    if (g == 2) affine_load(sn);
                    WN_M(X, 1, 0, 0, acc);
                    WN_ISSUE_PIECE((g + 2) % RING, 0);
                    WN_M(X, 1, 1, 0, acc);
                    WN_FENCE();
                    if (g == 2) { affine_math(0, 3); WN_FENCE(); }
                    else { conv_a(jn); WN_FENCE(); }
                    WN_M(X, 0, 0, 1, acc);
                    WN_FENCE();
                    if (g == 2) { affine_math(3, NIT); WN_FENCE(); }
                    else { conv_b(); WN_FENCE(); }
                    WN_M(X, 0, 1, 1, acc);
                    WN_FENCE();
                    if (g == 2) { conv_a(jn); conv_b(); WN_FENCE(); }
                    else { conv_c(); WN_FENCE(); }
                    WN_M(X, 0, 0, 0, acc);
                    WN_FENCE();
                    if (g == 2) { conv_c(); }
                    conv_d(nslo[jn]);
                    WN_FENCE();
                    WN_M(X, 0, 1, 0, acc);
                } else {
                    WN_PROD_A(X, acc);
                    WN_ISSUE_PIECE((g + 2) % RING, 0);
                    WN_PROD_B(X, acc);
                }
                WN_READ(X, slo[j], dz * WL::HY + 2, (g % RING) * GB + 2 * STEPB);
                if (!(g == 2 || g == 4 || g == 7 || g == 10)) {
                    __builtin_amdgcn_sched_group_barrier(0x008, 5, 0);
                    __builtin_amdgcn_sched_group_barrier(0x100, 6, 0);
                    __builtin_amdgcn_sched_group_barrier(0x008, 1, 0);
                }
                __builtin_amdgcn_sched_barrier(0);
                WN_PROD_A(Y, acc);
                WN_ISSUE_PIECE((g + 2) % RING, 1);
                WN_PROD_B(Y, acc);
                {
                    const int g1 = g + 1 < 12 ? g + 1 : 0;
                    const int so = g + 1 < 12 ? slo[g1 / 3] : nslo[0] * WL::SLOT;
                    WN_READ(Y, so, (g1 % 3) * WL::HY, ((g + 1) % RING) * GB);
                }
                __builtin_amdgcn_sched_group_barrier(0x008, 5, 0);
                __builtin_amdgcn_sched_group_barrier(0x100, 6, 0);
                __builtin_amdgcn_sched_group_barrier(0x008, 1, 0);
                __builtin_amdgcn_sched_barrier(0);
                WN_PROD_A(X, acc);
                WN_ISSUE_PIECE((g + 2) % RING, 2);
                WN_PROD_B(X, acc);
                if (g == 0) issue_rows(sn);
                __builtin_amdgcn_sched_barrier(0);
                if (dz == 2) {
                    WN_FLUSH(j, acc);
#pragma unroll
                    for (int u = 0; u < NT; ++u)
#pragma unroll
                        for (int q = 0; q < 16; ++q) acc[u][q] = 0.f;
                }
            }
            sbase = nbase;
        }
        GN_WAIT_VM_ONLY(2);
        __builtin_amdgcn_s_barrier();

        {
            int be = b, cbe = cb, z0e = z0, y0e = y0, x0e = x0, te = threadIdx.x;
            asm volatile("" : "+s"(be), "+s"(cbe), "+s"(z0e), "+s"(y0e), "+s"(x0e));
            asm volatile("" : "+v"(te));
            const int re = te & 31, he = (te >> 5) & 1;
            const int n0 = cbe * 128 + cg * 64;
            const int gz = z0e + zs;
            double ssum[NT], ssq[NT];
            float osc[NT], k63[NT];
#pragma unroll
            for (int u = 0; u < NT; ++u) { ssum[u] = 0.0; ssq[u] = 0.0; osc[u] = ecl[cg * 64 + u * 32 + re]; k63[u] = ecl[128 + cg * 64 + u * 32 + re]; }
            const bool interior = z0e > 0 && z0e + GN_CONV_TZ < p.D && y0e > 0 && y0e + GN_CONV_TY < p.H && x0e > 0 && x0e + GN_CONV_TX < p.W;
            const bool classes = p.kbias && !interior;
            const int mz = sp_axis_mask(gz, p.D);
            const float *const orow = p.out + ((((int64_t)be * p.D + gz) * p.H + y0e) * p.W + x0e) * p.Cout + n0;
            const int64_t rs2 = 2 * (int64_t)p.W * p.Cout;
#pragma unroll
            for (int e = 0; e < 2; ++e) {
                const int gy = y0e + he, gx = x0e + e;
                float kv[NT][16];
                if (classes) {
#pragma unroll
                    for (int u = 0; u < NT; ++u) {
                        const float *kb = p.kbias + (int64_t)be * 64 * p.Cout + n0 + u * 32 + re;
#pragma unroll
                        for (int q = 0; q < 16; ++q)
                            kv[u][q] = kb[(int64_t)((mz * 4 + sp_axis_mask(gy + 2 * (q >> 2), p.H)) * 4 + sp_axis_mask(gx + 2 * (q & 3), p.W)) * p.Cout];
                    }
                } else {
#pragma unroll
                    for (int u = 0; u < NT; ++u)
#pragma unroll
                        for (int q = 0; q < 16; ++q) kv[u][q] = k63[u];
                }
#pragma unroll
                for (int u = 0; u < NT; ++u) {
                    unsigned vo[4];
#pragma unroll
                    for (int i = 0; i < 4; ++i) vo[i] = (unsigned)(((he * p.W + e + 2 * i) * p.Cout + u * 32 + re) * 4);
#pragma unroll
                    for (int q = 0; q < 16; ++q) {
                        float v = __fmul_rn(tot[e][u][q], osc[u]);
                        if (p.kbias) v = __fadd_rn(v, kv[u][q]);
                        if (p.relu) v = gn_relu(v);
                        const float *ob = orow + (q >> 2) * rs2;
                        asm volatile("global_store_dword %0, %1, %2 nt" ::"v"(vo[q & 3]), "v"(v), "s"(ob) : "memory");
                        ssum[u] += (double)v;
                        ssq[u] += (double)v * (double)v;
                    }
                }
            }
            if (p.osum) {
#pragma unroll
                for (int u = 0; u < NT; ++u) {
                    const double s2 = ssum[u] + __shfl_xor(ssum[u], 32), q2 = ssq[u] + __shfl_xor(ssq[u], 32);
                    if (he == 0) {
                        const unsigned sa = (unsigned)(size_t)(__attribute__((address_space(3))) unsigned char *)smem + ST_OFF + (cg * 64 + u * 32 + re) * 8;
                        asm volatile("ds_add_f64 %0, %1\n\tds_add_f64 %0, %2 offset:1024" ::"v"(sa), "v"(s2), "v"(q2) : "memory");
                    }
                }
            }
        }
        if (!cont) {
            if (p.osum) {
                GN_WAIT_VM_LGKM0(63);
                __syncthreads();
                if (tid < 128) {
                    atomicAdd(&p.osum[(int64_t)b * p.Cout + cb * 128 + tid], stl[tid]);
                    atomicAdd(&p.osq[(int64_t)b * p.Cout + cb * 128 + tid], stl[128 + tid]);
                }
            }
            if (!more) break;
            fresh = true;
        }
        item = nitem; b = bn; cb = cbn; z0 = z0n; y0 = y0n; x0 = x0n;
    }
#undef WN_ISSUE_PIECE
#undef WN_M
#undef WN_FENCE
#undef WN_FLUSH
#undef WN_PROD_A
#undef WN_PROD_B
#undef WN_READ
    GN_WAIT_VM_LGKM0(0);
}

void gn_launch_conv3d_wino(const SplitArgs &p0, int tiles, hipStream_t st) {
    SplitArgs p = p0;
    const int64_t per_sample = (int64_t)tiles * (p.Cout / 128);
    int chain = (int)(per_sample / 64);
    chain = chain < 1 ? 1 : chain > 16 ? 16 : chain;
    if (const char *e = getenv("GARMENTNETS_WINO_CHAIN")) { const int forced = atoi(e); if (forced > 0 && forced <= 4096) chain = forced; }
    const int64_t items = per_sample * p.B;
    p.chain = chain;
    const int64_t span = 32 * (int64_t)chain;
    hipLaunchKernelGGL((conv3d_split_wino_kernel<true>), dim3((unsigned)((items + span - 1) / span * 32)), dim3(512), 0, st, p);
}
```

garmentnets_amd/csrc/unet_wino32.hip:

```cpp
#include "split_conv.h"

struct Wino32Layout {
    static constexpr int VB = 64;
    static constexpr int ROWP = 4 * VB + 16;
    static constexpr int TZ = 8, HZ = TZ + 2, HY = GN_CONV_TY + 2, ROWS = HZ * HY;
    static constexpr int SLOT = ROWS * ROWP;
    static constexpr int NSLOT = 5;
};

template <bool F16>
__global__ __launch_bounds__(512, 1) void conv3d_split_wino32pc_kernel(SplitArgs p) {
    constexpr int P = 2;
    using WL = Wino32Layout;
    constexpr int STEPB = P * 1024;
    constexpr int GB = 3 * STEPB;
    constexpr int RING = 4;
    constexpr int HALO_BYTES = WL::NSLOT * WL::SLOT;
    constexpr int AD_OFF = HALO_BYTES + RING * GB;
    constexpr int ADN = 128;
    constexpr int NIT = 10;
    constexpr int ST_OFF = AD_OFF + 2 * ADN * 4;
    constexpr int EC_OFF = ST_OFF + 2 * 32 * 8;
    __shared__ __attribute__((aligned(16))) unsigned char smem[EC_OFF + 2 * 32 * 4];
    const unsigned lds_ring = (unsigned)(size_t)(__attribute__((address_space(3))) unsigned char *)smem + HALO_BYTES;
    float *const adl = reinterpret_cast<float *>(smem + AD_OFF);
    const int tid = threadIdx.x, lane = tid & 63, h = lane >> 5, r = lane & 31;
    const int wave = __builtin_amdgcn_readfirstlane(tid >> 6);
    const bool consumer = wave < 4;
    const int cw = wave & 3;
    const int Cin = p.C0;
    const int ncb = p.Cout / 32;
    const int tiles_z = p.D / WL::TZ;
    const int tps = tiles_z * p.tiles_x * p.tiles_y;
    const int nslices = Cin / SP_KS;
    double *const stl = reinterpret_cast<double *>(smem + ST_OFF);
    float *const ecl = reinterpret_cast<float *>(smem + EC_OFF);

    const unsigned n_items = (p.active_list ? (unsigned)(*p.active_count) : (unsigned)(p.B * tps)) * (unsigned)ncb;
    const unsigned span = 32u * (unsigned)p.chain;
    const unsigned nch = (n_items + span - 1u) / span * 32u;
    if (blockIdx.x >= nch) return;
    const unsigned chn = (blockIdx.x & 7u) * (nch >> 3) + (blockIdx.x >> 3);
    int item = (int)((chn >> 5) * span + (chn & 31u));
    const int item_end = (int)(((chn >> 5) + 1u) * span < n_items ? ((chn >> 5) + 1u) * span : n_items);
    if (item >= item_end) return;
    auto decode = [&](int it, int &b_, int &cb_, int &z0_, int &y0_, int &x0_) {
        const int t = it / ncb;
        cb_ = it - t * ncb;
        const int e = p.active_list ? p.active_list[t] : t;
        b_ = e / tps;
        int tile = e - b_ * tps;
        const int tz = tile % tiles_z; tile /= tiles_z;
        const int tx = tile % p.tiles_x;
        z0_ = tz * WL::TZ; y0_ = (tile / p.tiles_x) * GN_CONV_TY; x0_ = tx * GN_CONV_TX;
    };
    int b, cb, z0, y0, x0;
    decode(item, b, cb, z0, y0, x0);

    f32x16 acc[2], tot[2][2];

    const int64_t bstep = (int64_t)ncb * STEPB;
    const unsigned char *bgs = nullptr;
    const unsigned bvoff = (unsigned)(lane * 16);
#define W32_PIECE(SLOTI, PI)                                                                                                   \
    gn_glds16_s(bgs + (int64_t)((PI) >> 1) * bstep + ((PI) & 1) * 1024, bvoff,                                                 \
                lds_ring + (SLOTI) * GB + (unsigned)(((PI) >> 1) * STEPB + ((PI) & 1) * 1024))
#define W32_ISSUE_GROUP(SLOTI)                                                                                                 \
    do {                                                                                                                       \
        W32_PIECE(SLOTI, cw);                                                                                                  \
        if (cw < 2) W32_PIECE(SLOTI, cw + 4);                                                                                  \
        bgs += 3 * bstep;                                                                                                      \
    } while (0)
#define W32_PRODUCER_WAIT(G)                                                                                                   \
    do {                                                                                                                       \
        const bool rows_ = (G) == 1 || (G) == 2;                                                                               \
        if (cw < 2) { if (rows_) GN_WAIT_VM_LGKM0(2 + 2 * NIT); else GN_WAIT_VM_LGKM0(2); }                                     \
        else if (cw == 2) { if (rows_) GN_WAIT_VM_LGKM0(1 + 2 * NIT); else GN_WAIT_VM_LGKM0(1); }                               \
        else { if (rows_) GN_WAIT_VM_LGKM0(1 + NIT); else GN_WAIT_VM_LGKM0(1); }                                                \
    } while (0)

    auto stage_row = [&](int t) {
        const int srow = (t >> 6) * 16 + 2 * ((t >> 2) & 3) + ((t >> 4) & 1) + 8 * ((t >> 5) & 1);
        return srow < WL::ROWS ? srow : WL::ROWS - 1;
    };
    const int pt = tid & 255;
    const bool two_tasks = cw < 3;
    const int c4 = (tid & 3) * 4;
    int wrow[2];
#pragma unroll
    for (int k = 0; k < 2; ++k) wrow[k] = stage_row(pt + 256 * k) * WL::ROWP + c4 * 2;
    unsigned voff1[2] = {0, 0}, voff0[2] = {0, 0}, voff9[2] = {0, 0}, inb[2] = {0, 0};
    auto set_rows = [&](int z0_, int y0_, int x0_) {
        int t = threadIdx.x & 255;
        asm volatile("" : "+v"(t));
        const int cq = (t & 3) * 4;
        const unsigned vs = (unsigned)p.C0 * 4u;
#pragma unroll
        for (int k = 0; k < 2; ++k) {
            const int rr = stage_row(t + 256 * k), hz = rr / WL::HY, hy = rr - hz * WL::HY;
            const int gz = z0_ + hz - 1, gy = y0_ + hy - 1;
            const bool rowin = gz >= 0 && gz < p.D && gy >= 0 && gy < p.H;
            voff1[k] = rowin ? ((unsigned)((gz * p.H + gy) * p.W + x0_) * (unsigned)p.C0 + (unsigned)cq) * 4u : (unsigned)cq * 4u;
            const bool in0 = rowin && x0_ - 1 >= 0, in9 = rowin && x0_ + 8 < p.W;
            voff0[k] = in0 ? voff1[k] - vs : voff1[k];
            voff9[k] = in9 ? voff1[k] + 8u * vs : voff1[k];
            inb[k] = rowin ? (0x1feu | (in0 ? 1u : 0u) | (in9 ? 0x200u : 0u)) : 0u;
        }
    };
    const float *base0 = p.src0;
    f32x4 raw[2][NIT];
    auto issue_rows = [&](int sl) {
        const unsigned cb4 = (unsigned)sl * (SP_KS * 4u), vs = (unsigned)p.C0 * 4u;
#pragma unroll
        for (int k = 0; k < 2; ++k) {
            if (k == 1 && !two_tasks) break;
#pragma unroll
            for (int v = 0; v < NIT; ++v) {
                const unsigned vo = (v == 0 ? voff0[k] : v == NIT - 1 ? voff9[k] : voff1[k] + (unsigned)(v - 1) * vs) + cb4;
                asm volatile("global_load_dwordx4 %0, %1, %2" : "=v"(raw[k][v]) : "v"(vo), "s"(base0) : "memory");
            }
        }
    };
    float4 afa, afd;
    auto affine_rows = [&](int sl) {
        afa = *reinterpret_cast<const float4 *>(adl + sl * SP_KS + c4);
        afd = *reinterpret_cast<const float4 *>(adl + ADN + sl * SP_KS + c4);
#pragma unroll
        for (int k = 0; k < 2; ++k) {
            if (k == 1 && !two_tasks) break;
#pragma unroll
            for (int v = 0; v < NIT; ++v) {
                asm volatile("" : "+v"(raw[k][v]));
                const bool in = (inb[k] >> v) & 1u;
                raw[k][v].x = in ? __fmaf_rn(raw[k][v].x, afa.x, afd.x) : 0.f;
                raw[k][v].y = in ? __fmaf_rn(raw[k][v].y, afa.y, afd.y) : 0.f;
                raw[k][v].z = in ? __fmaf_rn(raw[k][v].z, afa.z, afd.z) : 0.f;
                raw[k][v].w = in ? __fmaf_rn(raw[k][v].w, afa.w, afd.w) : 0.f;
            }
        }
    };
    auto convert = [&](int jp, int slot, int k0, int k1) {
#pragma unroll
        for (int k = 0; k < 2; ++k) {
            if (k == 1 && !two_tasks) break;
            unsigned char *dst = smem + slot * WL::SLOT + wrow[k];
#pragma unroll
            for (int q = k0; q < k1; ++q) {
                f32x4 cv;
                if (jp == 0) cv = raw[k][2 * q] - raw[k][2 * q + 2];
                else if (jp == 1) cv = raw[k][2 * q + 1] + raw[k][2 * q + 2];
                else if (jp == 2) cv = raw[k][2 * q + 2] - raw[k][2 * q + 1];
                else cv = raw[k][2 * q + 1] - raw[k][2 * q + 3];
                uint2 cp[P];
                split4<P, F16>(cv.x, cv.y, cv.z, cv.w, cp);
#pragma unroll
                for (int i = 0; i < P; ++i) *reinterpret_cast<uint2 *>(dst + q * WL::VB + i * 32) = cp[i];
            }
        }
    };

    const int abase = (2 * cw * WL::HY + (r >> 2)) * WL::ROWP + (r & 3) * WL::VB + 16 * h;
    const unsigned char *const ring_rd = smem + HALO_BYTES + lane * 16;
    uint4 fa[2][2][P], fb[2][P];
#define W32_READ(SET, SLOT_OFF, HROW, RING_OFF)                                                                                \
    do {                                                                                                                       \
        _Pragma("unroll") for (int f = 0; f < 2; ++f)                                                                          \
            _Pragma("unroll") for (int i = 0; i < P; ++i)                                                                      \
                fa[SET][f][i] = *reinterpret_cast<const uint4 *>(smem + (SLOT_OFF) + abase + ((HROW) + f * WL::HY) * WL::ROWP + i * 32); \
        _Pragma("unroll") for (int i = 0; i < P; ++i)                                                                          \
            fb[SET][i] = *reinterpret_cast<const uint4 *>(ring_rd + (RING_OFF) + i * 1024);                                     \
    } while (0)
#define W32_PROD(SET)                                                                                                          \
    do {                                                                                                                       \
        acc[0] = mfma16<F16>(fa[SET][0][1], fb[SET][0], acc[0]); acc[1] = mfma16<F16>(fa[SET][1][1], fb[SET][0], acc[1]);       \
        acc[0] = mfma16<F16>(fa[SET][0][0], fb[SET][1], acc[0]); acc[1] = mfma16<F16>(fa[SET][1][0], fb[SET][1], acc[1]);       \
        acc[0] = mfma16<F16>(fa[SET][0][0], fb[SET][0], acc[0]); acc[1] = mfma16<F16>(fa[SET][1][0], fb[SET][0], acc[1]);       \
    } while (0)
#define W32_FLUSH(J)                                                                                                           \
    do {                                                                                                                       \
        _Pragma("unroll") for (int f = 0; f < 2; ++f)                                                                          \
            _Pragma("unroll") for (int q = 0; q < 16; ++q) {                                                                   \
                const float m = acc[f][q];                                                                                     \
                if ((J) <= 2) tot[f][0][q] = __fadd_rn(tot[f][0][q], m);                                                       \
                if ((J) == 1) tot[f][1][q] = __fadd_rn(tot[f][1][q], m);                                                       \
                if ((J) >= 2) tot[f][1][q] = __fsub_rn(tot[f][1][q], m);                                                       \
                acc[f][q] = 0.f;                                                                                               \
            }                                                                                                                  \
    } while (0)

    if (consumer) {
        bool fresh = true;
        int sbase = 0;
        for (;;) {
            if (fresh) {
                GN_WAIT_VM_LGKM0(0);
                __syncthreads();
                {
                    int tf = threadIdx.x;
                    asm volatile("" : "+v"(tf));
                    if (tf < Cin) { adl[tf] = p.a[(int64_t)b * Cin + tf]; adl[ADN + tf] = p.d[(int64_t)b * Cin + tf]; }
                    if (tf < 64) stl[tf] = 0.0;
                    if (tf < 32) {
                        const float osn = p.out_scale[(int64_t)b * p.osc_bstride + cb * 32 + tf];
                        ecl[tf] = p.act_inv ? __fmul_rn(osn, p.act_inv[b]) : osn;
                        ecl[32 + tf] = p.kbias ? p.kbias[((int64_t)b * 64 + 63) * p.Cout + cb * 32 + tf] : 0.f;
                    }
                }
                GN_WAIT_VM_LGKM0(0);
                __syncthreads();
                __syncthreads();
                sbase = 0;
                W32_READ(0, 0, 0, 0);
                fresh = false;
            }
#pragma unroll
            for (int f = 0; f < 2; ++f)
#pragma unroll
                for (int q = 0; q < 16; ++q) { acc[f][q] = 0.f; tot[f][0][q] = 0.f; tot[f][1][q] = 0.f; }
            const int nitem = item + 32;
            const bool more = nitem < item_end;
            int bn = b, cbn = cb, z0n = z0, y0n = y0, x0n = x0;
            if (more) decode(nitem, bn, cbn, z0n, y0n, x0n);
            const bool cont = more && bn == b && cbn == cb;
            for (int s = 0; s < nslices; ++s) {
                const int nbase = sbase == 0 ? 4 : sbase - 1;
                int slo[4], nslo0;
#pragma unroll
                for (int j = 0; j < 4; ++j) { const int a_ = sbase + j; slo[j] = (a_ >= WL::NSLOT ? a_ - WL::NSLOT : a_) * WL::SLOT; }
                nslo0 = nbase * WL::SLOT;
#pragma unroll
                for (int g = 0; g < 12; ++g) {
                    const int j = g / 3, dz = g % 3, X = g & 1, Y = X ^ 1;
                    if (g > 0 || s > 0) __builtin_amdgcn_s_barrier();
                    W32_READ(Y, slo[j], dz * WL::HY + 1, (g % RING) * GB + STEPB);
                    W32_PROD(X);
                    W32_READ(X, slo[j], dz * WL::HY + 2, (g % RING) * GB + 2 * STEPB);
                    W32_PROD(Y);
                    {
                        const int g1 = g + 1 < 12 ? g + 1 : 0;
                        const int so = g + 1 < 12 ? slo[g1 / 3] : nslo0;
                        W32_READ(Y, so, (g1 % 3) * WL::HY, ((g + 1) % RING) * GB);
                    }
                    W32_PROD(X);
                    if (dz == 2) W32_FLUSH(j);
                }
                sbase = nbase;
            }
            __builtin_amdgcn_s_barrier();
            {
                int be = b, cbe = cb, z0e = z0, y0e = y0, x0e = x0, te = threadIdx.x;
                asm volatile("" : "+s"(be), "+s"(cbe), "+s"(z0e), "+s"(y0e), "+s"(x0e));
                asm volatile("" : "+v"(te));
                const int re = te & 31, he = (te >> 5) & 1;
                const int n0 = cbe * 32;
                double ssum = 0.0, ssq = 0.0;
                const float osc = ecl[re], k63 = ecl[32 + re];
                const bool interior = z0e > 0 && z0e + WL::TZ < p.D && y0e > 0 && y0e + GN_CONV_TY < p.H && x0e > 0 && x0e + GN_CONV_TX < p.W;
                const bool classes = p.kbias && !interior;
                const int64_t rs2 = 2 * (int64_t)p.W * p.Cout;
#pragma unroll
                for (int f = 0; f < 2; ++f) {
                    const int gz = z0e + 2 * cw + f;
                    const int mz = sp_axis_mask(gz, p.D);
                    const float *const orow = p.out + ((((int64_t)be * p.D + gz) * p.H + y0e) * p.W + x0e) * p.Cout + n0;
                    const float *prow = nullptr;
// ... 151 lines not shown
```

garmentnets_amd/ops.py:

```python
import ctypes
import math
import threading

import numpy as np
import torch

from . import _lib

_i32 = torch.int32


class _CallState(threading.local):
    dev = None


_CALL = _CallState()


def _stream():
    dev, _CALL.dev = _CALL.dev, None
    if dev is not None and dev.index is not None and dev.index != torch.cuda.current_device():
        torch.cuda.set_device(dev)
    return ctypes.c_void_p(torch.cuda.current_stream(dev).cuda_stream)

# ... 197 lines not shown


def _i3(v):
    return (ctypes.c_int * 3)(*[int(a) for a in v])


def grid_features(feat, nocs, sim_pos, conf, batch, lower, upper, grid_shape, include_point=True, include_conf=True):
    N, Cf = feat.shape
    C = Cf + (6 if include_point else 0) + (3 if include_conf else 0)
    out = new_rows(N, C, feat.device)
    flat = torch.empty(N, dtype=_i32, device=feat.device)
    _lib.call("gn_grid_features", _p(feat), rows_view(feat)[1], Cf, _p(_chk(nocs, torch.float32, "nocs")),
              _p(_chk(sim_pos, torch.float32, "sim_pos")), _p(_chk(conf, torch.float32, "conf")), _p(_chk(batch, torch.int64, "batch")),
              N, _f3(lower), _f3(upper), _i3(grid_shape), 1 if include_point else 0, 1 if include_conf else 0, _p(out),
              out.stride(0), _p(flat), _stream())
    return out, flat


def zeroed_volume(B, grid_shape, C, device):
    vol = torch.zeros((B,) + tuple(grid_shape) + (C,), dtype=torch.float32, device=device)
    cnt = torch.zeros(B * int(np.prod(grid_shape)), dtype=_i32, device=device)
    return vol, cnt


REDUCE_CODES = {"max": 0, "mean": 1, "sum": 2, "add": 2, "min": 3, "mul": 4}


def grid_scatter(src, flat_idx, B, grid_shape, reduce, with_stats=False, prezeroed=None, c_real=None):
    N, C = src.shape
    if reduce not in REDUCE_CODES:
        raise ValueError(f"grid_scatter: reduce={reduce!r} is not one of {sorted(REDUCE_CODES)}")
    if with_stats and reduce == "mul":
        raise ValueError("grid_scatter: the occupied-cell statistics assume empty cells are 0, which 'mul' leaves at 1")
    cps = int(np.prod(grid_shape))
    cells = B * cps
    if prezeroed is not None:
        vol, cnt = prezeroed
        assert vol.shape == (B,) + tuple(grid_shape) + (C,) and cnt.numel() == cells
    else:
        vol = torch.empty((B,) + tuple(grid_shape) + (C,), dtype=torch.float32, device=src.device)
        cnt = torch.empty(cells, dtype=_i32, device=src.device)
    code = REDUCE_CODES[reduce]
    nbytes = _lib.load().gn_grid_scatter_workspace_bytes(N, C, code)
    ws = torch.empty(nbytes, dtype=torch.uint8, device=src.device) if nbytes else None
    _lib.call("gn_grid_scatter_ex", _p(src), rows_view(src)[1], _p(flat_idx), N, C, C if c_real is None else int(c_real), cells, code, _p(vol), _p(cnt),
              _p(ws), nbytes, 0 if prezeroed is None else 1, _stream())
    if not with_stats:
        return vol
    s, q = _stats_buffers(B, C, src.device, True)
    _lib.call("gn_grid_stats", _p(vol), _p(flat_idx), N, C, cps, B, _p(cnt), _p(s), _p(q), _stream())
    return vol, (s, q, cps)


def channel_stats(x):
    B, C = x.shape[0], x.shape[-1]
    V = x.numel() // (B * C)
    s, q = _stats_buffers(B, C, x.device, True)
    narrow = (C <= 256 and 256 % C == 0) or C % 256 == 0
    _lib.call("gn_channel_stats" if narrow else "gn_channel_stats_any", _p(x), B, V, C, _p(s), _p(q), _stream())
    return s, q, V


def groupnorm_affine(st0, st1, groups, eps, gamma, beta, with_act_scale=False, real=None):
    s0, q0, V0 = st0
    B, C0 = s0.shape
    if st1 is not None:
        s1, q1, V1 = st1
        C1 = s1.shape[1]
        rep = V0 // V1
    else:
        s1 = q1 = None
        C1, V1, rep = 0, 0, 1
    a = torch.empty((B, C0 + C1), dtype=torch.float32, device=s0.device)
    d = torch.empty_like(a)
    inv = torch.empty(B, dtype=torch.float32, device=s0.device) if with_act_scale else None
    r0, r1 = (C0, C1) if real is None else (int(real[0]), int(real[1]) if len(real) > 1 else 0)
    if (r0, r1) == (C0, C1) and C0 + C1 <= GNA_MAXC:
        _lib.call("gn_groupnorm_affine", _p(s0), _p(q0), C0, V0, _p(s1), _p(q1), C1, V1, rep, B, groups, float(eps), _p(gamma), _p(beta),
                  _p(a), _p(d), _p(inv), _stream())
    else:
        _lib.call("gn_groupnorm_affine_map", _p(s0), _p(q0), r0, C0, V0, _p(s1), _p(q1), r1, C1, V1, rep, B, groups, float(eps), _p(gamma),
                  _p(beta), _p(a), _p(d), _p(inv), _stream())
    return (a, d, inv) if with_act_scale else (a, d)


GNA_MAXC = 1024


def pack_conv_weight(w):
    cout, cin = w.shape[:2]
    assert cin % 16 == 0
    return w.detach().float().permute(2, 3, 4, 1, 0).reshape(27, cin // 16, 16, cout).permute(0, 1, 3, 2).contiguous()


from .arith import CONV_FP32, CONV_MODE_NAMES, SPLIT_BF16X2, SPLIT_BF16X3, SPLIT_F16X2


class SplitPack:

    def __init__(self, tensor, mode, out_scale):
        self.tensor, self.mode, self.out_scale = tensor, int(mode), out_scale

    def to(self, device):
        return SplitPack(self.tensor.to(device), self.mode, self.out_scale.to(device))


def pack_conv_weight_split(w, mode):
    if mode not in (SPLIT_BF16X2, SPLIT_BF16X3, SPLIT_F16X2):
        raise ValueError(f"unknown split mode {mode}")
    cout, cin = w.shape[:2]
    w = w.detach().float()
    planes, dt = (2, torch.float16) if mode == SPLIT_F16X2 else (int(mode), torch.bfloat16)
    scale = torch.ones(cout, dtype=torch.float32)
    if mode == SPLIT_F16X2:
        m = w.reshape(cout, -1).abs().amax(dim=1).cpu()
        ok = torch.isfinite(m) & (m > 0)
        scale = torch.where(ok, torch.exp2(-torch.floor(torch.log2(torch.where(ok, m, torch.ones_like(m))))), scale).float()
    base = (w * scale.to(w.device).view(cout, 1, 1, 1, 1)).permute(2, 3, 4, 1, 0).reshape(27, cin // 16, 2, 8, cout // 32, 32)
    base = base.permute(1, 0, 4, 2, 5, 3)
    out, r = [], base
    for _ in range(planes):
        p = r.to(dt)
        out.append(p)
        r = r - p.float()
    pk = torch.stack(out, dim=3).contiguous()
    pk = pk.reshape(cin // 16 * 27, -1)
    pk = torch.cat([pk, torch.zeros_like(pk[:1]).repeat(8, 1)], dim=0)
    return SplitPack(pk.contiguous().view(torch.int16), mode, (1.0 / scale).contiguous().to(w.device))


def wino_supported(cin, cout, dims):
    D, H, W = [int(v) for v in dims]
    if not (cin % 16 == 0 and cout % 32 == 0 and H % 8 == 0 and W % 8 == 0 and D * H * W <= (1 << 27) and D * H * W * cin * 4 < (1 << 32)):
        return False
    return (cin <= 256 and D % 4 == 0) if cout % 128 == 0 else (cin <= 128 and D % 8 == 0)


def pack_conv_weight_split_wino(w):
    cout, cin = w.shape[:2]
    w = w.detach().double().cpu()
    G = torch.tensor([[1.0, 0.0, 0.0], [0.5, 0.5, 0.5], [0.5, -0.5, 0.5], [0.0, 0.0, 1.0]], dtype=torch.float64)
    u = torch.einsum("jk,nczyk->nczyj", G, w)
    m = u.reshape(cout, -1).abs().amax(dim=1)
    scale = _pow2_floor_inv(m)
    base = (u * scale.view(cout, 1, 1, 1, 1)).float().permute(4, 2, 3, 1, 0).reshape(36, cin // 16, 2, 8, cout // 32, 32)
    base = base.permute(1, 0, 4, 2, 5, 3)
    p1 = base.to(torch.float16)
    p2 = (base - p1.float()).to(torch.float16)
    pk = torch.stack((p1, p2), dim=3).contiguous().reshape(cin // 16 * 36, -1)
    pk = torch.cat([pk, torch.zeros_like(pk[:6])], dim=0)
    return SplitPack(pk.contiguous().view(torch.int16), SPLIT_F16X2, (1.0 / scale).float().contiguous())


def conv3d_gcr_split_wino(src, a, d, pack, cout, relu=True, with_stats=False, act_inv=None, tile_active=None, kconst=None, kreach=1, partial=None):
    return _conv3d_wino("conv3d_gcr_split_wino", src, a, d, pack.tensor, pack.out_scale, act_inv, None, cout, relu, with_stats, tile_active, kconst, kreach,
                        partial)


def _conv3d_wino(who, src, a, d, pack, out_scale, act_inv, kbias, cout, relu, with_stats, tile_active, kconst, kreach, partial):
    B, D, H, W, C0 = src.shape
    out = torch.empty((B, D, H, W, cout), dtype=torch.float32, device=src.device)
    s, q = _stats_buffers(B, cout, src.device, with_stats)
    if partial is not None:
        if tile_active is not None:
            raise ValueError(f"{who}: the occupancy-aware launch cannot take a polyphase partial")
        _lib.call("gn_conv3d_gcr_split_wino_partial", _p(src), C0, _p(a), _p(d), _p(pack), _p(out_scale), _p(act_inv), _p(kbias), B, D, H, W, cout,
                  1 if relu else 0, _p(out), _p(s), _p(q), _p(_chk(partial, torch.float32, "partial")), _stream())
    else:
        ows, ows_bytes = _occupancy_ws(tile_active, B, D, H, W, src.device)
        _lib.call("gn_conv3d_gcr_split_wino", _p(src), C0, _p(a), _p(d), _p(pack), _p(out_scale), _p(act_inv), _p(kbias), B, D, H, W, cout,
                  1 if relu else 0, _p(out), _p(s), _p(q), _p(tile_active), _p(kconst), int(kreach), _p(ows), ows_bytes, _stream())
    return (out, (s, q, D * H * W)) if with_stats else out


def grid_tile_flags(flat_idx, B, grid_shape, reach=1):
    g0, g1, g2 = [int(v) for v in grid_shape]
    tiles = -(-g0 // 4) * -(-g1 // 8) * -(-g2 // 8)
    flags = torch.empty((B, tiles), dtype=torch.uint8, device=flat_idx.device)
    _lib.call("gn_grid_tile_flags", _p(_chk(flat_idx, _i32, "flat_idx")), flat_idx.numel(), B, g0, g1, g2, int(reach), _p(flags), _stream())
    return flags


def polyphase_weights(w, c0):
    w = w.detach().double().cpu()
    cout = w.shape[0]
    w0, w1 = w[:, :c0].float(), w[:, c0:]
    M = torch.zeros(2, 3, 3, dtype=torch.float64)
    M[0, 0, 0] = M[0, 1, 1] = M[0, 1, 2] = 1.0
    M[1, 1, 0] = M[1, 1, 1] = M[1, 2, 2] = 1.0
    blocks = [torch.einsum("az,by,cx,nkzyx->nkabc", M[pz], M[py], M[px], w1) for pz in (0, 1) for py in (0, 1) for px in (0, 1)]
    wm = torch.cat(blocks, dim=0).float()
    nz = (wm.reshape(8 * cout // 32, 32, -1, 27) != 0).any(dim=2).any(dim=1)
    mask = torch.zeros(27, dtype=torch.int64)
    for blk in range(nz.shape[0]):
        mask |= nz[blk].to(torch.int64) << blk
    return w0.contiguous(), wm.contiguous(), mask.to(torch.int32)


def pack_upconv_weight(wm, cout, mode):
    if mode not in (SPLIT_BF16X2, SPLIT_F16X2):
        raise ValueError("gn_upconv_partial runs the two-plane modes only")
    wm = wm.detach().float().cpu()
    c1 = wm.shape[1]
    assert wm.shape[0] == 8 * cout and c1 % 16 == 0 and cout % 32 == 0
    taps = torch.empty((8, 8, cout, c1), dtype=torch.float32)
    for c in range(8):
        pz, py, px = c >> 2, (c >> 1) & 1, c & 1
        for t in range(8):
            iz, iy, ix = t >> 2, (t >> 1) & 1, t & 1
            taps[c, t] = wm[c * cout:(c + 1) * cout, :, pz + iz, py + iy, px + ix]
    scale = torch.ones(8, cout)
    if mode == SPLIT_F16X2:
        m = taps.abs().amax(dim=(1, 3))
        ok = torch.isfinite(m) & (m > 0)
        scale = torch.where(ok, torch.exp2(-torch.floor(torch.log2(torch.where(ok, m, torch.ones_like(m))))), scale)
    dt = torch.float16 if mode == SPLIT_F16X2 else torch.bfloat16
    t_ = (taps * scale[:, None, :, None]).reshape(8, 8, cout // 32, 32, c1 // 16, 2, 8)
    t_ = t_.permute(4, 1, 0, 2, 5, 3, 6)
    p1 = t_.to(dt)
    p2 = (t_ - p1.float()).to(dt)
    pk = torch.stack((p1, p2), dim=4).contiguous()
    return SplitPack(pk.view(torch.int16).reshape(-1), mode, (1.0 / scale).reshape(-1).contiguous())


def _device_pack_args(who, w, c_lo, c_n):
    if not isinstance(w, torch.Tensor) or w.dim() != 5 or tuple(w.shape[2:]) != (3, 3, 3):
        raise ValueError(f"{who}: expected a Conv3d weight (Cout, Cin, 3, 3, 3)")
    if w.dtype != torch.float32:
        raise ValueError(f"{who}: expected torch.float32, got {w.dtype}")
    if not w.is_contiguous():
        raise ValueError(f"{who}: the weight must be contiguous")
    cout, cin = int(w.shape[0]), int(w.shape[1])
    c_lo = int(c_lo)
    c_n = cin - c_lo if c_n is None else int(c_n)
    if c_lo < 0 or c_n <= 0 or c_lo + c_n > cin:
        raise ValueError(f"{who}: input channels [{c_lo}, {c_lo + c_n}) outside the weight's {cin}")
    if c_n % 16 != 0 or cout % 32 != 0:
        raise ValueError(f"{who}: channels must be multiples of 16 (in) / 32 (out), got {c_n} / {cout}")
    if not w.is_cuda:
        raise ValueError(f"{who}: the weight must be on the GPU (the host builder takes a CPU tensor)")
    return w.detach(), cout, cin, c_lo, c_n


def pack_conv_weight_split_device(w, mode, c_lo=0, c_n=None):
    if mode not in (SPLIT_BF16X2, SPLIT_BF16X3, SPLIT_F16X2):
        raise ValueError(f"unknown split mode {mode}")
    w, cout, cin, c_lo, c_n = _device_pack_args("pack_conv_weight_split_device", w, c_lo, c_n)
    planes = 2 if mode == SPLIT_F16X2 else int(mode)
    pk = torch.empty((c_n // 16 * 27 + 8, cout // 32 * planes * 512), dtype=torch.int16, device=w.device)
    scale = torch.empty((cout,), dtype=torch.float32, device=w.device)
    _lib.call("gn_weight_pack_split", _p(w), cout, cin, c_lo, c_n, int(mode), _p(pk), pk.numel() * 2, _p(scale), _stream())
    return SplitPack(pk, mode, scale)


def pack_conv_weight_split_wino_device(w, c_lo=0, c_n=None):
    w, cout, cin, c_lo, c_n = _device_pack_args("pack_conv_weight_split_wino_device", w, c_lo, c_n)
    pk = torch.empty((c_n // 16 * 36 + 6, cout // 32 * 2 * 512), dtype=torch.int16, device=w.device)
    scale = torch.empty((cout,), dtype=torch.float32, device=w.device)
    _lib.call("gn_weight_pack_split_wino", _p(w), cout, cin, c_lo, c_n, _p(pk), pk.numel() * 2, _p(scale), _stream())
    return SplitPack(pk, SPLIT_F16X2, scale)


def pack_upconv_weight_device(w, c0, mode):
    if mode not in (SPLIT_BF16X2, SPLIT_F16X2):
        raise ValueError("gn_upconv_partial runs the two-plane modes only")
    w, cout, cin, c0, c1 = _device_pack_args("pack_upconv_weight_device", w, c0, None)
    pk = torch.empty((c1 // 16 * 64 * (cout // 32) * 2 * 512,), dtype=torch.int16, device=w.device)
    scale = torch.empty((8 * cout,), dtype=torch.float32, device=w.device)
    _lib.call("gn_weight_pack_upconv", _p(w), cout, cin, c0, int(mode), _p(pk), pk.numel() * 2, _p(scale), _stream())
    return SplitPack(pk, mode, scale)


def upconv_partial(src1, a1, d1, pack, cout, act_inv=None):
    B, Dc, Hc, Wc, C1 = src1.shape
    part = torch.empty((B, Dc, Hc, Wc, 8 * cout), dtype=torch.float32, device=src1.device)
    _lib.call("gn_upconv_partial", _p(src1), C1, _p(_chk(a1, torch.float32, "a")), _p(_chk(d1, torch.float32, "d")), _p(pack.tensor), pack.mode,
              _p(pack.out_scale), _p(act_inv), B, Dc, Hc, Wc, cout, _p(part), _stream())
    return part


def conv3d_gcr_split(src0, src1, a, d, pack, cout, relu=True, with_stats=False, act_inv=None, tile_active=None, kconst=None, kreach=1,
                     partial=None):
    B, D, H, W, C0 = src0.shape
    C1 = 0 if src1 is None else src1.shape[-1]
    out = torch.empty((B, D, H, W, cout), dtype=torch.float32, device=src0.device)
    s, q = _stats_buffers(B, cout, src0.device, with_stats)
    ows, ows_bytes = _occupancy_ws(tile_active, B, D, H, W, src0.device)
    _lib.call("gn_conv3d_gcr_split", _p(src0), C0, _p(src1), C1, _p(a), _p(d), _p(pack.tensor), pack.mode, _p(pack.out_scale), _p(act_inv), B, D, H, W, cout,
              1 if relu else 0, _p(out), _p(s), _p(q), _p(tile_active), _p(kconst), int(kreach), _p(partial), _p(ows), ows_bytes, _stream())
    return (out, (s, q, D * H * W)) if with_stats else out


class AffinePack:
    __slots__ = ("pack", "stage_a", "stage_d", "out_scale", "kbias", "cin", "cout", "wino")


def conv_affine_pack(weight, a, d, stats, rest=None, wino=False):
    cout, cin = int(weight.shape[0]), int(weight.shape[1])
    B, dev = a.shape[0], a.device
    w = weight.detach()
    _chk(w, torch.float32, "weight")
    _chk(a, torch.float32, "a"); _chk(d, torch.float32, "d")
    if rest is not None:
        _chk(rest, torch.float32, "rest")
        assert tuple(rest.shape) == (B, cin)
    sfx = "_wino" if wino else ""
    nbytes = getattr(_lib.load(), "gn_conv_affine_pack" + sfx + "_bytes")(B, cin, cout)
    if nbytes == 0 and B > 0:
        raise ValueError("conv_affine_pack: channel counts must be multiples of 16 (in) / 32 (out)")
    r = AffinePack()
    r.cin, r.cout, r.wino = cin, cout, bool(wino)
    r.pack = torch.empty((max(nbytes, 16),), dtype=torch.uint8, device=dev)
    r.stage_a = torch.empty((B, cin), dtype=torch.float32, device=dev)
    r.stage_d = torch.empty((B, cin), dtype=torch.float32, device=dev)
    r.out_scale = torch.empty((B, cout), dtype=torch.float32, device=dev)
    r.kbias = torch.empty((B, 64, cout), dtype=torch.float32, device=dev)
    ws = torch.empty((B * cin * 12 + B * cout * 4 + 16,), dtype=torch.uint8, device=dev)
    _lib.call("gn_conv_affine_pack" + sfx, _p(w), cin, cout, _p(a), _p(d), _p(stats[0]), _p(stats[1]), int(stats[2]), _p(rest), B, _p(r.pack), nbytes,
              _p(r.stage_a), _p(r.stage_d), _p(r.out_scale), _p(r.kbias), _p(ws), ws.numel(), _stream())
    return r


def conv3d_gcr_split_persample(src, prep, relu=True, with_stats=False, tile_active=None, kconst=None, kreach=1, partial=None):
    B, D, H, W, C = src.shape
    assert C == prep.cin and B == prep.stage_a.shape[0]
    if prep.wino:
        return _conv3d_wino("conv3d_gcr_split_persample", src, prep.stage_a, prep.stage_d, prep.pack, prep.out_scale, None, prep.kbias, prep.cout, relu,
                            with_stats, tile_active, kconst, kreach, partial)
    out = torch.empty((B, D, H, W, prep.cout), dtype=torch.float32, device=src.device)
    s, q = _stats_buffers(B, prep.cout, src.device, with_stats)
    ows, ows_bytes = _occupancy_ws(tile_active, B, D, H, W, src.device)
    _lib.call("gn_conv3d_gcr_split_persample", _p(src), C, _p(prep.stage_a), _p(prep.stage_d), _p(prep.pack), _p(prep.out_scale), _p(prep.kbias),
              B, D, H, W, prep.cout, 1 if relu else 0, _p(out), _p(s), _p(q), _p(tile_active), _p(kconst), int(kreach), _p(partial), _p(ows), ows_bytes,
              _stream())
    return (out, (s, q, D * H * W)) if with_stats else out


def _occupancy_ws(tile_active, B, D, H, W, device):
    if tile_active is None:
        return None, 0
    n = _lib.load().gn_conv3d_occupancy_workspace_bytes(B, D, H, W)
    return torch.empty((n,), dtype=torch.uint8, device=device), n


def _stats_buffers(B, C, device, want):
    if not want:
        return None, None
    sq = torch.empty((2, B, C), dtype=torch.float64, device=device)
    return sq[0], sq[1]


def conv3d_gcr(src0, src1, a, d, wp, cout, relu=True, with_stats=False):
    B, D, H, W, C0 = src0.shape
    C1 = 0 if src1 is None else src1.shape[-1]
    out = torch.empty((B, D, H, W, cout), dtype=torch.float32, device=src0.device)
    s, q = _stats_buffers(B, cout, src0.device, with_stats)
    _lib.call("gn_conv3d_gcr", _p(src0), C0, _p(src1), C1, _p(a), _p(d), _p(wp), B, D, H, W, cout, 1 if relu else 0, _p(out),
              _p(s), _p(q), _stream())
    return (out, (s, q, D * H * W)) if with_stats else out


ACT_NONE, ACT_RELU, ACT_LEAKY, ACT_ELU = 0, 1, 2, 3


def affine_act(x, a=None, d=None, bias=None, act=ACT_NONE, out=None):
    B, C = x.shape[0], x.shape[-1]
    V = x.numel() // max(B * C, 1)
    if out is None:
        out = torch.empty_like(x)
    _lib.call("gn_affine_act", _p(x), B, V, C, _p(a), _p(d), _p(bias), int(act), _p(out), _stream())
    return out


def maxpool3d_2(x, with_stats=False):
    B, D, H, W, C = x.shape
    out = torch.empty((B, D // 2, H // 2, W // 2, C), dtype=torch.float32, device=x.device)
    epilogue = with_stats and 0 < C <= 256 and C % 4 == 0 and 256 % (C // 4) == 0
    s, q = _stats_buffers(B, C, x.device, epilogue)
    _lib.call("gn_maxpool3d_2", _p(x), B, D, H, W, C, _p(out), _p(s), _p(q), _stream())
    if with_stats and not epilogue:
        return out, channel_stats(out)
    return (out, (s, q, (D // 2) * (H // 2) * (W // 2))) if with_stats else out


def trilinear_sample(vol_b, query=None, Q=0, m0=0, M=None, out=None):
    D, H, W, C = _chk(vol_b, torch.float32, "vol_b").shape
    if query is not None:
        M = query.shape[0]
        _chk(query, torch.float32, "query")
    if out is None:
        out = new_rows(M, C, vol_b.device)
    elif out.dtype != torch.float32:
        raise TypeError(f"out: expected {torch.float32}, got {out.dtype}")
    _lib.call("gn_trilinear_sample", _p(vol_b), D, H, W, C, _p(query), int(Q), int(m0), int(M), _p(out), rows_view(out)[1], _stream())
    return out


def pack_kpair(w):
    n, k = w.shape
    assert k % 16 == 0
    return w.detach().float().reshape(n, k // 16, 2, 8).permute(1, 0, 2, 3).contiguous()


def implicit_decode(vol_b, layers, query=None, Q=0, m0=0, M=None, out=None, xin=None, run_if=None):
    (w1p, b1, s1, t1, N1), (w2p, b2, s2, t2, N2), (w3, b3, s3, t3, OUT) = layers
    if xin is not None:
        if xin.dtype != torch.float32:
            raise TypeError(f"xin: expected {torch.float32}, got {xin.dtype}")
        D = H = W = 0
        M, C0 = xin.shape
        ldxin = rows_view(xin)[1]
        vol_b = None
    else:
        D, H, W, C0 = _chk(vol_b, torch.float32, "vol_b").shape
        ldxin = 0
    if query is not None:
        M = query.shape[0]
        _chk(query, torch.float32, "query")
    if out is None:
        out = torch.empty((M, OUT), dtype=torch.float32, device=(xin if xin is not None else vol_b).device)
    elif out.dtype != torch.float32:
        raise TypeError(f"out: expected {torch.float32}, got {out.dtype}")
    _lib.call("gn_implicit_decode", _p(vol_b), D, H, W, C0, _p(xin), ldxin, _p(query), int(Q), int(m0), int(M), _p(w1p), _p(b1), _p(s1), _p(t1), N1,
              _p(w2p), _p(b2), _p(s2), _p(t2), N2, _p(w3), _p(b3), _p(s3), _p(t3), OUT, _p(out), rows_view(out)[1], _p(run_if), _stream())
    return out


def _chk_row_sets(t, name):
    if t.dtype != torch.float32:
        raise TypeError(f"{name}: expected {torch.float32}, got {t.dtype}")
    if t.dim() == 3 and t.numel() == 0:
        return t
    if t.dim() != 3 or (t.shape[2] > 1 and t.stride(2) != 1) or (t.shape[0] > 1 and t.stride(0) != t.shape[1] * t.stride(1)):
        raise ValueError(f"{name}: need (B, M, C) rows of unit stride, the row sets packed back to back")
    return t


def trilinear_sample_batch(vol, query, out=None):
    B, D, H, W, C = vol.shape
    M = query.shape[1]
    _chk(vol, torch.float32, "vol")
    _chk(query, torch.float32, "query")
    if out is None:
        out = torch.empty((B, M, pad4(C)), dtype=torch.float32, device=vol.device)[:, :, :C]
    _chk_row_sets(out, "out")
    _lib.call("gn_trilinear_sample_batch", _p(vol), B, vol.stride(0), D, H, W, C, _p(query), int(M), _p(out), out.stride(1), _stream())
    return out


def implicit_decode_batch(xin, layers, out, run_if=None, run_if_stride=0):
    (w1p, b1, s1, t1, N1), (w2p, b2, s2, t2, N2), (w3, b3, s3, t3, OUT) = layers
    B, M, C0 = _chk_row_sets(xin, "xin").shape
    _chk_row_sets(out, "out")
    _lib.call("gn_implicit_decode_batch", _p(xin), xin.stride(1), int(M), B, C0, _p(w1p), _p(b1), _p(s1), _p(t1), N1, _p(w2p), _p(b2), _p(s2), _p(t2), N2,
              _p(w3), _p(b3), _p(s3), _p(t3), OUT, _p(out), out.stride(1), _p(run_if), int(run_if_stride), _stream())
    return out


def implicit_decode_split_batch(xin, pack, out, xscale=None):
    B, M, C0 = xin.shape
    assert xin.stride(0) == M * xin.stride(1) and out.stride(0) == M * out.stride(1), "row sets must be packed back to back"
    _lib.call("gn_implicit_decode_split_batch", _p(xin), xin.stride(1), int(M), B, _p(pack.wpack), _p(pack.tab), _p(xscale),
              C0, pack.hidden, pack.hidden, pack.out_channels, _p(out), out.stride(1), _stream())
    return out


class DecodeSplitPack:

    def __init__(self, wpack, tab, smax, out_channels, hidden=256):
        self.wpack, self.tab, self.smax, self.out_channels, self.hidden = wpack, tab, float(smax), int(out_channels), int(hidden)

    def to(self, device):
        return DecodeSplitPack(self.wpack.to(device), self.tab.to(device), self.smax, self.out_channels, self.hidden)


def _pow2_floor_inv(m):
    ok = torch.isfinite(m) & (m > 0)
    return torch.where(ok, torch.exp2(-torch.floor(torch.log2(torch.where(ok, m, torch.ones_like(m))))), torch.ones_like(m))


def _d_unit(q, h):
    return (q & 3) + 8 * (q >> 2) + 4 * h


def pack_decode_split(layers):
    (w1, b1, s1, t1), (w2, b2, s2, t2), (w3, b3, s3, t3) = layers
    dd = lambda v, n, fill: (torch.full((n,), fill, dtype=torch.float64) if v is None else v.detach().double().cpu())
    w1, w2, w3 = w1.detach().double().cpu(), w2.detach().double().cpu(), w3.detach().double().cpu()
    out_c, N = w3.shape[0], w2.shape[0]
    assert N in (256, 512) and w1.shape[0] == N and w2.shape == (N, N) and w3.shape[1] == N and 1 <= out_c <= 4
    assert w1.shape[1] in ((128, 32) if N == 256 else (32,)), "the 512-wide pack takes the folded 32-channel first layer"
    k0g, npair, nb_, kg2 = w1.shape[1] // 16, N // 64, N // 32, N // 16
    b2f = dd(b2, N, 0.0) + w2 @ dd(t1, N, 0.0)
    w2 = w2 * dd(s1, N, 1.0)[None, :]
    b3f = (dd(b3, out_c, 0.0) + w3 @ dd(t2, N, 0.0)).float()
    w3 = w3 * dd(s2, N, 1.0)[None, :]
    b1f = dd(b1, N, 0.0)
    r1 = _pow2_floor_inv(w1.abs().amax(dim=1))
    w1s, b1s = (w1 * r1[:, None]).float(), (b1f * r1).float()
    w2 = w2 / r1[None, :]
    r2 = _pow2_floor_inv(w2.abs().amax(dim=1))
    w2s, b2s = (w2 * r2[:, None]).float(), (b2f * r2).float()
    w3s = (w3 / r2[None, :]).float()
    bmax = max(float(b1s.abs().max()), float(b2s.abs().max()))
    smax = 2.0 ** 60 if not (bmax > 0 and math.isfinite(bmax)) else min(2.0 ** 60, 2.0 ** math.floor(math.log2(8192.0 / bmax)))
# ... 1194 lines not shown
```

include/garmentnets_hip.h:

```cpp
#ifndef GARMENTNETS_HIP_H
#define GARMENTNETS_HIP_H

#include <stddef.h>
#include <stdint.h>

#ifdef __cplusplus
extern "C" {
#endif

#define GN_OK 0
#define GN_EINVAL (-1)
#define GN_ELAUNCH (-2)
#define GN_ECAP (-3)

const char *gn_last_error(void);
int gn_version(void);
const char *gn_last_kernel(void);
int gn_device_info(int *num_cu, int *lds_bytes_per_cu);


int gn_segment_ptr(const int64_t *batch, int64_t n, int B, int32_t *ptr, void *stream);

int gn_fps(const float *pos, const int32_t *ptr, const int32_t *out_ptr, const int32_t *start_idx, int B,
           int max_points_per_example, int32_t *out_idx, void *stream);

int gn_fps_nested(const float *pos, const int32_t *ptr, const int32_t *out_ptr, const int32_t *start_idx, int B,
                  int max_points_per_example, int32_t *out_idx, float *gap_out, const float *nested_gap, void *stream);
size_t gn_fps_workspace_bytes(int B, int max_points_per_example);
int gn_fps_nested_ws(const float *pos, const int32_t *ptr, const int32_t *out_ptr, const int32_t *start_idx, int B,
                     int max_points_per_example, int32_t *out_idx, float *gap_out, const float *nested_gap, void *ws, size_t ws_bytes,
                     void *stream);

int gn_ball_query(const float *pos, const int32_t *ptr, const int32_t *centre_idx, const int32_t *centre_ptr, int B,
                  int M, float r2, int K, int32_t *nbr, int32_t *cnt, void *stream);

int gn_sa_gather(const float *x, int ldx, int C, const float *pos, const int32_t *centre_idx, const int32_t *nbr,
                 int M, int K, int self_loops, float *out, int ldo, int32_t *slot_src, void *stream);
int gn_sa_gather_scoped(const float *x, int ldx, int C, const float *pos, const int32_t *centre_idx, const int32_t *nbr,
                        int M, int K, int self_loops, const int32_t *self_src, float *out, int ldo, int32_t *slot_src, void *stream);

int gn_segment_max(const float *in, int ldi, const int32_t *slot_src, int M, int S, int C, float *out, int ldo,
                   void *stream);

int gn_sa_fused_supported(int C, int N1, int N2, int N3);
int gn_sa_fused(const float *x, int ldx, int C, const float *pos, const int32_t *centre_idx, const int32_t *nbr, const int32_t *cnt,
                int M, int K, int self_loops, const float *w1p, const float *w2p, const float *w3p, const float *tab, int N1, int N2,
                int N3, float *out, int ldo, void *stream);
int gn_sa_fused_scoped(const float *x, int ldx, int C, const float *pos, const int32_t *centre_idx, const int32_t *nbr, const int32_t *cnt,
                       int M, int K, int self_loops, const int32_t *self_src, const float *w1p, const float *w2p, const float *w3p,
                       const float *tab, int N1, int N2, int N3, float *out, int ldo, void *stream);
int gn_sa_fused_group(const float *x, int ldx, int C, const float *pos, const int32_t *centre_idx, const int32_t *nbr, const int32_t *cnt,
                      int M, int K, int self_loops, const int32_t *self_src, const float *w1p, const float *w2p, const float *w3p,
                      const float *tab, int N1, int N2, int N3, float *out, int ldo, void *stream, int group);
int gn_sa_fused_auto_group(int C, int N1, int N2, int N3, int M);

int gn_global_max_pool(const float *in, int ldi, const int32_t *ptr, int B, int C, float *out, int ldo, void *stream);

int gn_knn_interpolate(const float *xs, int ldx, const float *ps, const int32_t *ptr_s, const float *pq,
                       const int32_t *ptr_q, int B, int Nq, int C, int k, float *out, int ldo, void *stream);
int gn_knn_interpolate_any(const float *xs, int ldx, const float *ps, const int32_t *ptr_s, const float *pq,
                           const int32_t *ptr_q, int B, int Nq, int C, int k, float *out, int ldo, void *stream);

int gn_linear(const float *X, int ldx, const float *W, int ldw, const float *bias, const float *bn_scale,
              const float *bn_shift, int relu, int64_t M, int N, int K, float *Y, int ldy, void *stream);

int gn_nocs_head(const float *logits, int ldl, int64_t N, int bins, int64_t *bin_idx , float *confidence ,
                 float *pred_nocs , void *stream);


int gn_grid_features(const float *feat, int ldf, int Cf, const float *nocs, const float *sim_pos, const float *conf,
                     const int64_t *batch, int64_t N, const float lower[3], const float upper[3], const int grid[3],
                     int include_point, int include_conf, float *out, int ldo, int32_t *flat_idx, void *stream);

size_t gn_grid_scatter_workspace_bytes(int64_t N, int C, int reduce);
int gn_grid_scatter(const float *src, int lds, const int32_t *flat_idx, int64_t N, int C, int64_t cells, int reduce,
                    float *vol, int32_t *count_ws, void *ws, size_t ws_bytes, int vol_is_zeroed, void *stream);
int gn_grid_scatter_ex(const float *src, int lds, const int32_t *flat_idx, int64_t N, int C, int c_real, int64_t cells, int reduce,
                       float *vol, int32_t *count_ws, void *ws, size_t ws_bytes, int vol_is_zeroed, void *stream);

int gn_grid_tile_flags(const int32_t *flat_idx, int64_t N, int B, int G0, int G1, int G2, int reach, unsigned char *flags, void *stream);

int gn_grid_stats(const float *vol, const int32_t *flat_idx, int64_t N, int C, int64_t cells_per_sample, int B,
                  int32_t *count_ws, double *sum, double *sumsq, void *stream);


int gn_channel_stats(const float *x, int B, int64_t V, int C, double *sum, double *sumsq, void *stream);

int gn_channel_stats_any(const float *x, int B, int64_t V, int C, double *sum, double *sumsq, void *stream);

int gn_groupnorm_affine(const double *sum0, const double *sq0, int C0, int64_t V0, const double *sum1, const double *sq1,
                        int C1, int64_t V1, int rep1, int B, int groups, float eps, const float *gamma,
                        const float *beta, float *a, float *d, float *act_inv_scale, void *stream);

int gn_groupnorm_affine_map(const double *sum0, const double *sq0, int C0, int S0, int64_t V0, const double *sum1, const double *sq1,
                            int C1, int S1, int64_t V1, int rep1, int B, int groups, float eps, const float *gamma,
                            const float *beta, float *a, float *d, float *act_inv_scale, void *stream);

int gn_conv3d_gcr(const float *src0, int C0, const float *src1, int C1, const float *a, const float *d,
                  const float *wp, int B, int D, int H, int W, int Cout, int relu, float *out, double *out_sum,
                  double *out_sumsq, void *stream);

#define GN_SPLIT_BF16X2 2
#define GN_SPLIT_BF16X3 3
#define GN_SPLIT_F16X2 4
size_t gn_conv3d_occupancy_workspace_bytes(int B, int D, int H, int W);
int gn_conv3d_gcr_split(const float *src0, int C0, const float *src1, int C1, const float *a, const float *d,
                        const void *wp_planes, int mode, const float *out_scale, const float *act_inv_scale, int B, int D, int H, int W,
                        int Cout, int relu, float *out, double *out_sum, double *out_sumsq, const unsigned char *tile_active,
                        const float *kconst, int kreach, const float *partial, void *occ_ws, size_t occ_ws_bytes, void *stream);

size_t gn_conv_affine_pack_bytes(int B, int Cin, int Cout);
int gn_conv_affine_pack(const float *w, int Cin, int Cout, const float *a, const float *d, const double *sum, const double *sumsq, int64_t V,
                        const float *coff, int B, void *pack, size_t pack_bytes, float *stage_a, float *stage_d, float *out_scale,
                        float *kbias, void *ws, size_t ws_bytes, void *stream);
int gn_conv3d_gcr_split_persample(const float *src, int Cin, const float *stage_a, const float *stage_d, const void *pack,
                                  const float *out_scale, const float *kbias, int B, int D, int H, int W, int Cout, int relu, float *out,
                                  double *out_sum, double *out_sumsq, const unsigned char *tile_active, const float *kconst, int kreach,
                                  const float *partial, void *occ_ws, size_t occ_ws_bytes, void *stream);

size_t gn_conv_affine_pack_wino_bytes(int B, int Cin, int Cout);
int gn_conv_affine_pack_wino(const float *w, int Cin, int Cout, const float *a, const float *d, const double *sum, const double *sumsq, int64_t V,
                             const float *coff, int B, void *pack, size_t pack_bytes, float *stage_a, float *stage_d, float *out_scale,
                             float *kbias, void *ws, size_t ws_bytes, void *stream);
int gn_conv3d_gcr_split_wino(const float *src, int Cin, const float *a, const float *d, const void *pack, const float *out_scale,
                             const float *act_inv_scale, const float *kbias, int B, int D, int H, int W, int Cout, int relu, float *out,
                             double *out_sum, double *out_sumsq, const unsigned char *tile_active, const float *kconst, int kreach,
                             void *occ_ws, size_t occ_ws_bytes, void *stream);
int gn_conv3d_gcr_split_wino_partial(const float *src, int Cin, const float *a, const float *d, const void *pack, const float *out_scale,
                                     const float *act_inv_scale, const float *kbias, int B, int D, int H, int W, int Cout, int relu, float *out,
                                     double *out_sum, double *out_sumsq, const float *partial, void *stream);

int gn_upconv_partial(const float *src1, int C1, const float *a, const float *d, const void *wp, int mode, const float *out_scale,
                      const float *act_inv_scale, int B, int Dc, int Hc, int Wc, int Cout, float *partial, void *stream);

size_t gn_weight_pack_split_bytes(int c_n, int Cout, int mode);
size_t gn_weight_pack_split_wino_bytes(int c_n, int Cout);
size_t gn_weight_pack_upconv_bytes(int C1, int Cout);
int gn_weight_pack_split(const float *w, int Cout, int Cin, int c_lo, int c_n, int mode, void *pack, size_t pack_bytes, float *out_scale,
                         void *stream);
int gn_weight_pack_split_wino(const float *w, int Cout, int Cin, int c_lo, int c_n, void *pack, size_t pack_bytes, float *out_scale,
                              void *stream);
int gn_weight_pack_upconv(const float *w, int Cout, int Cin, int c0, int mode, void *pack, size_t pack_bytes, float *out_scale, void *stream);

int gn_affine_act(const float *x, int B, int64_t V, int C, const float *a, const float *d, const float *bias, int act, float *out, void *stream);

int gn_maxpool3d_2(const float *in, int B, int D, int H, int W, int C, float *out, double *out_sum, double *out_sumsq,
                   void *stream);

int gn_trilinear_sample(const float *vol, int D, int H, int W, int C, const float *query, int Q, int64_t m0, int64_t M,
                        float *out, int ldo, void *stream);
int gn_trilinear_sample_batch(const float *vol, int B, int64_t vol_bstride, int D, int H, int W, int C, const float *query, int64_t M, float *out, int ldo,
                              void *stream);

int gn_implicit_decode(const float *vol, int D, int H, int W, int C0, const float *xin, int ldxin, const float *query, int Q, int64_t m0, int64_t M,
                       const float *w1p, const float *b1, const float *s1, const float *t1, int N1, const float *w2p,
                       const float *b2, const float *s2, const float *t2, int N2, const float *w3, const float *b3,
                       const float *s3, const float *t3, int OUT, float *out, int ldo, const float *run_if, void *stream);


int gn_ggm3d(const float *vol, int n0, int n1, int n2, double sigma, float *tmp, float *out, void *stream);

int gn_minmax(const float *x, int64_t n, float *out2, void *stream);
int gn_ggm3d_batch(const float *vol, int batch, int n0, int n1, int n2, double sigma, float *tmp, float *out, void *stream);
int gn_minmax_batch(const float *x, int batch, int64_t n, float *out2, void *stream);
size_t gn_ggm3d_range_workspace_bytes(int batch, int n0, int n1, int n2);
int gn_ggm3d_batch_ex(const float *vol, int batch, int n0, int n1, int n2, double sigma, float *tmp, float *out, int accum_bits, float *range2,
                      void *range_ws, size_t range_ws_bytes, void *stream);

size_t gn_mc33_workspace_bytes(int n0, int n1, int n2);
int gn_mc33(const float *vol, int n0, int n1, int n2, double level, void *ws, size_t ws_bytes, float *verts,
            int32_t *faces, float *normals, float *values, int64_t cap_v, int64_t cap_f, int64_t *counts_dev,
            void *stream);
size_t gn_mc33_batch_workspace_bytes(int batch, int n0, int n1, int n2);
int gn_mc33_batch(const float *vol, int batch, int n0, int n1, int n2, double level, void *ws, size_t ws_bytes, float *verts,
                  int32_t *faces, float *normals, float *values, int64_t cap_v, int64_t cap_f, int64_t *counts_dev, void *stream);
int gn_mc33_batch_profiled(const float *vol, int batch, int n0, int n1, int n2, double level, void *ws, size_t ws_bytes, float *verts,
                           int32_t *faces, float *normals, float *values, int64_t cap_v, int64_t cap_f, int64_t *counts_dev, void *stream,
                           float *stage_ms);

int gn_gather_nn(const float *vol, int n0, int n1, int n2, const float *verts_vox, int64_t nv, double spacing,
                 float *out, void *stream);
int gn_gather_nn_batch(const float *vol, int batch, int n0, int n1, int n2, const float *verts_vox, int64_t nv, double spacing,
                       float *out, void *stream);

int gn_scale_verts(const float *verts_vox, int64_t nv, double spacing, float *verts_out, void *stream);

size_t gn_mesh_compact_workspace_bytes(int64_t V, int64_t F);
int gn_mesh_compact(const void *verts, int vert_bytes, const int32_t *faces, const unsigned char *on_surface, int64_t V, int64_t F,
                    void *ws, size_t ws_bytes, void *out_verts, int32_t *out_faces, int64_t *counts, void *stream);

size_t gn_mesh_largest_component_workspace_bytes(int64_t V);
int gn_mesh_largest_component(const int32_t *faces, int64_t F, int64_t V, void *ws, size_t ws_bytes, unsigned char *mask, int32_t *label,
                              int64_t *info, void *stream);

int gn_implicit_decode_split(const float *xin, int ldxin, int64_t M, const void *wpack, const float *tab, const float *xscale,
                             int C0, int N1, int N2, int OUT, float *out, int ldo, void *stream);
int gn_implicit_decode_split_batch(const float *xin, int ldxin, int64_t M, int B, const void *wpack, const float *tab, const float *xscale,
                                   int C0, int N1, int N2, int OUT, float *out, int ldo, void *stream);
int gn_implicit_decode_batch(const float *xin, int ldxin, int64_t M, int B, int C0, const float *w1p, const float *b1, const float *s1, const float *t1,
                             int N1, const float *w2p, const float *b2, const float *s2, const float *t2, int N2, const float *w3, const float *b3,
                             const float *s3, const float *t3, int OUT, float *out, int ldo, const float *run_if, int run_if_stride, void *stream);

int gn_implicit_decode_lattice_split(const float *vol, int D, int H, int W, int C0, int Q, int64_t m0, int64_t M, const void *wpack,
                                     const float *tab, const float *xscale, int N1, int N2, int OUT, float *out, int ldo, void *stream);

int gn_decoder_input_scale(const double *sumsq, int64_t V, int B, int C, float smax, float *out4, void *stream);


int gn_nearest_neighbor(const float *query, int64_t nq, const float *ref, int64_t nr, int32_t *idx, float *d2, void *stream);

int gn_nearest_neighbor_f64_batch(const double *query, const double *ref, const int64_t *pairs, int P, int64_t max_nq, int32_t *idx, double *d2,
                                  void *stream);

int gn_point_mesh_sqdist_batch(const double *query, const double *verts, const int32_t *faces, const int64_t *pairs, int P, int64_t max_nq,
                               int32_t *face_idx, double *d2, int64_t *bad, void *stream);


int gn_winding_number_batch(const double *query, const double *verts, const int32_t *faces, const int64_t *pairs, int P, int64_t max_nq,
                            double *out, int64_t *bad, void *stream);

int gn_winding_field_batch(const double *verts, const int32_t *faces, const int64_t *mesh_csr, int B, int D, int H, int W, float *out,
                           int64_t *bad, void *stream);

int gn_distance_field_batch(const double *verts, const int32_t *faces, const int64_t *mesh_csr, int B, int D, int H, int W,
                            int32_t *face_idx, double *d2, int64_t *bad, void *stream);

#define GN_QT_FACE_CHUNK 512
#define GN_QT_WINDING 0
#define GN_QT_DISTANCE 1
#define GN_QT_SIGNED_DISTANCE 2
#define GN_QT_OCCUPANCY 3

int gn_query_targets_face_chunk(void);
size_t gn_query_targets_workspace_bytes(int B, int64_t M, int64_t max_nf, int kind);
int gn_query_targets_batch(const float *query, const float *verts, const int32_t *faces, const int64_t *mesh_csr, int B, int64_t M, int64_t max_nf, int kind,
                           int use_clip, float tsdf_clip, int absolute, void *ws, size_t ws_bytes, float *target, double *w, double *d2, int32_t *face_idx,
                           int64_t *bad, void *stream);

#define GN_LOSS_MAX_SETS 8
#define GN_LOSS_L2 0
#define GN_LOSS_SMOOTH_L1 1
#define GN_LOSS_BCE_LOGITS 2
#define GN_LOSS_ROW_NORM 3

typedef struct {
    const float *logits;
    const float *gt;
    int64_t n;
    int ldl;
    int pad;
} GnNocsBinSet;

typedef struct {
    const float *pred;
    const float *target;
    int64_t count;
    int kind;
    int mirror;
} GnLossSegment;

size_t gn_nocs_bin_metrics_workspace_bytes(const GnNocsBinSet *sets_host, int nsets);
int gn_nocs_bin_metrics(const GnNocsBinSet *sets_host, int nsets, int bins, int mirror_axis, void *ws, size_t ws_bytes, double *out, void *stream);

size_t gn_value_losses_workspace_bytes(const GnLossSegment *segs_host, int nsegs);
int gn_value_losses(const GnLossSegment *segs_host, int nsegs, void *ws, size_t ws_bytes, double *out, void *stream);

typedef struct {
    const float *logits;
    const float *gt;
    float *grad;
    int64_t n;
    int ldl;
    int ldg;
    int ncols;
    int pad;
} GnNocsBinGradSet;

typedef struct {
    const float *pred;
    const float *target;
    float *grad;
    int64_t count;
    double coef;
// ... 195 lines not shown
```

Baseline: 157.9.

## Pass channel-blocked intermediate between paired Winograd convs in UNet blocks

Adds a channel-blocked layout (16-channel slabs, spatial-major within each slab) for the intermediate tensor of a double-conv block. The 128-wide Winograd kernel writes it when Cout is a multiple of 128, and the 32-wide Winograd kernel reads it directly. The goal is more contiguous, cache-friendly staging loads in the second conv, whose per-slice reads were strided by the full channel count. This is gated on f16x2 mode, dense Winograd launches on both sides, and no gradients. It adds a new entry point, layout-tagged tensors and guards against misuse.

```diff
diff --git a/garmentnets_amd/_lib.py b/garmentnets_amd/_lib.py
--- a/garmentnets_amd/_lib.py
+++ b/garmentnets_amd/_lib.py
@@ -49,6 +49,7 @@
     "gn_conv_affine_pack_wino": [_vp, _i32, _i32, _vp, _vp, _vp, _vp, _i64, _vp, _i32, _vp, _sz, _vp, _vp, _vp, _vp, _vp, _sz, _vp],
     "gn_conv3d_gcr_split_wino": [_vp, _i32, _vp, _vp, _vp, _vp, _vp, _vp, _i32, _i32, _i32, _i32, _i32, _i32, _vp, _vp, _vp, _vp, _vp, _i32, _vp, _sz, _vp],
     "gn_conv3d_gcr_split_wino_partial": [_vp, _i32, _vp, _vp, _vp, _vp, _vp, _vp, _i32, _i32, _i32, _i32, _i32, _i32, _vp, _vp, _vp, _vp, _vp],
+    "gn_conv3d_gcr_split_wino_blocked": [_vp, _i32, _vp, _vp, _vp, _vp, _vp, _vp, _i32, _i32, _i32, _i32, _i32, _i32, _vp, _vp, _vp, _i32, _i32, _vp],
     "gn_weight_pack_split_bytes": [_i32, _i32, _i32],
     "gn_weight_pack_split_wino_bytes": [_i32, _i32],
     "gn_weight_pack_upconv_bytes": [_i32, _i32],
diff --git a/garmentnets_amd/arith.py b/garmentnets_amd/arith.py
--- a/garmentnets_amd/arith.py
+++ b/garmentnets_amd/arith.py
@@ -26,6 +26,7 @@
     affine_in_weights: bool = True
     winograd: bool = True
     winograd32: bool = True
+    blocked_mid: bool = True
     polyphase_upconv: bool = True
     fold_final_conv: bool = True
     fused_lattice: bool = True
@@ -55,7 +56,8 @@
         return cls(conv_mode=CONV_MODE_NAMES[_env_choice("GARMENTNETS_CONV_MODE", "f16x2", CONV_MODE_NAMES)],
                    decode_mode=_env_choice("GARMENTNETS_DECODE_MODE", "f16x2", DECODE_MODES),
                    sparse_first_conv=_env_flag("GARMENTNETS_SPARSE_CONV"), affine_in_weights=_env_flag("GARMENTNETS_AFFINE_IN_WEIGHTS"),
-                   winograd=_env_flag("GARMENTNETS_WINOGRAD"), winograd32=_env_flag("GARMENTNETS_WINOGRAD32"), polyphase_upconv=_env_flag("GARMENTNETS_POLYPHASE"),
+                   winograd=_env_flag("GARMENTNETS_WINOGRAD"), winograd32=_env_flag("GARMENTNETS_WINOGRAD32"),
+                   blocked_mid=_env_flag("GARMENTNETS_BLOCKED_MID"), polyphase_upconv=_env_flag("GARMENTNETS_POLYPHASE"),
                    fold_final_conv=_env_flag("GARMENTNETS_FOLD_FINAL_CONV"), fused_lattice=_env_flag("GARMENTNETS_FUSED_LATTICE"),
                    ggm_fp32=_env_flag("GARMENTNETS_GGM_FP32", False), device_packs=_env_flag("GARMENTNETS_DEVICE_PACKS", False),
                    conv_grad_mode=_env_choice("GARMENTNETS_CONV_GRAD_MODE", "fp32", CONV_GRAD_MODES))
diff --git a/garmentnets_amd/components/unet3d.py b/garmentnets_amd/components/unet3d.py
--- a/garmentnets_amd/components/unet3d.py
+++ b/garmentnets_amd/components/unet3d.py
@@ -69,6 +69,20 @@
            and min(dims) > 2 * reach and (reach == 1 or small is not None)
            and (not wino or small is None or ops.wino_supported(c0, cout, small)))
     return ConvPlan(mode, bool(aiw), bool(wino), bool(poly), (int(small[0]) if small is not None else 8 if wino else 5) if occ else 0)
+
+
+def block_plans(arith, dims, c0, c1, c_mid, cout, sparse=False, rest0=False):
+    if not sparse or c1:
+        return conv_plan(arith, dims, c0, c1, c_mid, rest0=rest0), conv_plan(arith, dims, c_mid, 0, cout)
+    p1 = conv_plan(arith, dims, c0, 0, c_mid, 1, False, None, True)
+    if not (p1.aiw or p1.small):
+        return p1, conv_plan(arith, dims, c_mid, 0, cout)
+    return p1, conv_plan(arith, dims, c_mid, 0, cout, 2, p1.aiw, (p1.small,) * 3 if p1.small else None, True)
+
+
+def mid_blocked(arith, p1, p2, c_mid, cout, grad=False, readers=1):
+    return bool(arith.blocked_mid and not grad and readers == 1 and p1.mode == ops.SPLIT_F16X2 and p2.mode == ops.SPLIT_F16X2
+                and p1.wino and not p1.poly and c_mid % 128 == 0 and p2.wino and not p2.poly and cout % 128 != 0 and not p1.small and not p2.small)
 
 
 class ConvGradPlan(NamedTuple):
@@ -209,15 +223,17 @@
                 ops.affine_act(y, a=na, d=nd, out=y)
         return y, (ops.channel_stats(y) if with_stats else None)
 
-    def run(self, src0, src1=None, stats0=None, stats1=None, with_stats=True, arith=None, rest0=None):
-        return self._run(src0, src1, stats0, stats1, with_stats, arith, None, rest0)[:2]
-
-    def run_at_rest(self, src0, at_rest, stats0=None, with_stats=True, arith=None):
-        return self._run(src0, None, stats0, None, with_stats, arith, at_rest, None)
-
-    def _run(self, src0, src1, stats0, stats1, with_stats, arith, at_rest, rest0):
+    def run(self, src0, src1=None, stats0=None, stats1=None, with_stats=True, arith=None, rest0=None, out_blocked=False):
+        return self._run(src0, src1, stats0, stats1, with_stats, arith, None, rest0, out_blocked)[:2]
+
+    def run_at_rest(self, src0, at_rest, stats0=None, with_stats=True, arith=None, out_blocked=False):
+        return self._run(src0, None, stats0, None, with_stats, arith, at_rest, None, out_blocked)
+
+    def _run(self, src0, src1, stats0, stats1, with_stats, arith, at_rest, rest0, out_blocked=False):
         arith = arith or AR.DEFAULT
         lay = self._layout(src0, src1)
+        if (out_blocked and self.order != "gcr") or (ops.is_blocked(src0) and (self.order != "gcr" or stats0 is None)):
+            raise RuntimeError("SingleConv: a channel-blocked tensor goes from one fused 'gcr' launch to the next, with its producer's statistics")
         if self.order != "gcr":
             return self._run_generic(src0, src1, stats0, stats1, with_stats, lay) + (None,)
         wp, gamma, beta = self.packed()
@@ -229,16 +245,19 @@
         reach, value, small, flat = (0, None, None, None) if at_rest is None else (at_rest.reach, at_rest.value, at_rest.small, at_rest.flat)
         plan = conv_plan(arith, tuple(src0.shape[1:4]), src0.shape[-1], 0 if src1 is None else src1.shape[-1], cout, reach, value is not None,
                          None if small is None else tuple(small.shape[1:4]), flat is not None, rest0 is not None)
+        if out_blocked and not (plan.wino and cout % 128 == 0 and not plan.small):
+            raise RuntimeError(f"SingleConv: a channel-blocked output was asked of a launch that cannot store one ({plan})")
         if plan.mode == ops.CONV_FP32:
             a, d = ops.groupnorm_affine(st0, st1, self.groupnorm.num_groups, self.groupnorm.eps, gamma, beta, real=None if lay is None else lay.real)
             if lay is not None:
                 wp = param_cache(self, "_split_packs").get(self._gen(lay), "fp32", lambda: ops.pack_conv_weight(self._padded_weight(lay)))
             r, nxt = ops.conv3d_gcr(src0, src1, a, d, wp, cout, relu=True, with_stats=with_stats), None
         else:
-            r, nxt = self._run_split(plan, src0, src1, st0, st1, with_stats, at_rest, gamma, beta, rest0, lay, device_packs=arith.device_packs)
+            r, nxt = self._run_split(plan, src0, src1, st0, st1, with_stats, at_rest, gamma, beta, rest0, lay, device_packs=arith.device_packs,
+                                      out_blocked=out_blocked)
         return (r + (nxt,)) if with_stats else (r, None, nxt)
 
-    def _run_split(self, plan, src0, src1, st0, st1, with_stats, at_rest, gamma, beta, rest0, lay=None, device_packs=False):
+    def _run_split(self, plan, src0, src1, st0, st1, with_stats, at_rest, gamma, beta, rest0, lay=None, device_packs=False, out_blocked=False):
         gn, weight, cout, mode, c0 = self.groupnorm, self.conv.weight, self.conv.out_channels, plan.mode, src0.shape[-1]
         real = None
         if lay is not None:
@@ -302,6 +321,8 @@
             B, n, reach = src0.shape[0], plan.small, at_rest.reach
             small_out = launch(at_rest.small if at_rest.small is not None else torch.zeros((B, n, n, n, c0), dtype=torch.float32, device=src0.device))
             occ = dict(tile_active=ops.grid_tile_flags(at_rest.flat, B, src0.shape[1:4], reach), kconst=_class_constants(small_out, reach, cout), kreach=reach)
+        if out_blocked:
+            occ = dict(occ, out_blocked=True)
         r = launch(src0, with_stats=with_stats, partial=part, **occ)
         learned = rest_out is not None or small_out is not None
         return r, (AtRest(at_rest.flat, at_rest.reach + 1, rest_out, small_out) if learned else None)
@@ -323,12 +344,22 @@
         self.SingleConv2.in_real = (c2_in,)
 
     def run(self, src0, src1=None, stats0=None, stats1=None, sparse_flat=None, arith=None, rest0=None):
+        blocked = self._mid_blocked(src0, src1, sparse_flat is not None, rest0 is not None, arith or AR.DEFAULT)
         if sparse_flat is None or src1 is not None:
-            y, st = self.SingleConv1.run(src0, src1, stats0, stats1, arith=arith, rest0=rest0)
+            y, st = self.SingleConv1.run(src0, src1, stats0, stats1, arith=arith, rest0=rest0, out_blocked=blocked)
             return self.SingleConv2.run(y, None, st, arith=arith) + (None,)
-        y, st, at_rest = self.SingleConv1.run_at_rest(src0, AtRest(sparse_flat, 1), stats0, arith=arith)
+        y, st, at_rest = self.SingleConv1.run_at_rest(src0, AtRest(sparse_flat, 1), stats0, arith=arith, out_blocked=blocked)
         y, st, at_rest = self.SingleConv2.run_at_rest(y, at_rest, st, arith=arith)
         return y, st, (None if at_rest is None else at_rest.value)
+
+    def _mid_blocked(self, src0, src1, sparse, rest0, arith):
+        c1, c2 = self.SingleConv1, self.SingleConv2
+        if c1.order != "gcr" or c2.order != "gcr":
+            return False
+        c_mid, cout = stored_channels(c1.conv.out_channels), stored_channels(c2.conv.out_channels)
+        p1, p2 = block_plans(arith, tuple(src0.shape[1:4]), src0.shape[-1], 0 if src1 is None else src1.shape[-1], c_mid, cout, sparse, rest0)
+        grad = torch.is_grad_enabled() and (src0.requires_grad or any(p.requires_grad for p in self.parameters()))
+        return mid_blocked(arith, p1, p2, c_mid, cout, grad=grad, readers=1)
 
 
 class Encoder(nn.Module):
diff --git a/garmentnets_amd/csrc/split_conv.h b/garmentnets_amd/csrc/split_conv.h
--- a/garmentnets_amd/csrc/split_conv.h
+++ b/garmentnets_amd/csrc/split_conv.h
@@ -28,6 +28,7 @@
     int osc_bstride;
     int kreach;
     int chain;
+    int src_blocked, out_blocked;
 };
 
 __device__ __forceinline__ bool sp_work_item(const SplitArgs &p, int ncb, int tiles_per_sample, int &b, int &tile, int &cb) {
diff --git a/garmentnets_amd/csrc/unet_split.hip b/garmentnets_amd/csrc/unet_split.hip
--- a/garmentnets_amd/csrc/unet_split.hip
+++ b/garmentnets_amd/csrc/unet_split.hip
@@ -861,7 +861,7 @@
                                  const void *wp_planes, int mode, const float *out_scale, const float *act_inv_scale, int B, int D, int H,
                                  int W, int Cout, int relu, float *out, double *out_sum, double *out_sumsq, const unsigned char *tile_active,
                                  const float *kconst, int kreach, const float *partial, const float *kbias, int64_t wp_bstride, int osc_bstride,
-                                 void *occ_ws, size_t occ_ws_bytes, void *stream, int wino = 0) {
+                                 void *occ_ws, size_t occ_ws_bytes, void *stream, int wino = 0, int src_blocked = 0, int out_blocked = 0) {
     GN_REQUIRE(B >= 0 && D > 0 && H > 0 && W > 0 && C0 > 0 && C1 >= 0 && Cout > 0, "gn_conv3d_gcr_split: bad sizes");
     GN_REQUIRE(mode == GN_SPLIT_BF16X2 || mode == GN_SPLIT_BF16X3 || mode == GN_SPLIT_F16X2, "gn_conv3d_gcr_split: mode must be GN_SPLIT_BF16X2, _BF16X3 or _F16X2");
     GN_REQUIRE(out_scale != nullptr, "gn_conv3d_gcr_split: out_scale [Cout] is required (ones for the bf16 modes)");
@@ -878,6 +878,7 @@
     p.C0 = C0; p.C1 = C1; p.B = B; p.D = D; p.H = H; p.W = W; p.Cout = Cout; p.relu = relu; p.out_scale = out_scale; p.act_inv = act_inv_scale;
     p.active_list = nullptr; p.active_count = nullptr; p.kconst = kconst; p.kreach = kreach; p.partial = partial;
     p.kbias = kbias; p.wp_bstride = wp_bstride; p.osc_bstride = osc_bstride; p.chain = 1;
+    p.src_blocked = src_blocked; p.out_blocked = out_blocked;
     GN_REQUIRE(!partial || (D % 2 == 0 && H % 2 == 0 && W % 2 == 0), "gn_conv3d_gcr_split: a polyphase partial needs even dims");
     const int tz = (int)gn_cdiv(D, GN_CONV_TZ);
     p.tiles_y = (int)gn_cdiv(H, GN_CONV_TY);
@@ -893,6 +894,8 @@
                "D*H*W*Cin*4 < 2^32");
     GN_REQUIRE(!wino32 || (mode == GN_SPLIT_F16X2 && C1 == 0 && C0 <= 128 && fits32 && D % 8 == 0 && H % 8 == 0 && W % 8 == 0 && (int64_t)D * H * W <= ((int64_t)1 << 27)),
                "gn_conv3d_gcr_split_wino (Cout %% 128 != 0): needs one source, Cin <= 128, D %% 8 == H %% 8 == W %% 8 == 0, D*H*W <= 2^27 and D*H*W*Cin*4 < 2^32");
+    GN_REQUIRE(!src_blocked || (wino32 && !tile_active), "gn_conv3d_gcr_split_wino_blocked: a channel-blocked source is read by the 32-wide Winograd kernel's dense launch alone");
+    GN_REQUIRE(!out_blocked || (wino && !wino32 && !tile_active), "gn_conv3d_gcr_split_wino_blocked: a channel-blocked output is written by the 128-wide Winograd kernel's dense launch alone");
     const int tiles8 = (int)gn_cdiv(D, 8) * p.tiles_y * p.tiles_x;
     const bool strip = !wino && mode != GN_SPLIT_BF16X3 && !wide128 && C1 == 0 && (int64_t)tiles8 * (Cout / 32) * B >= 512;
     const bool wide = !wino && !wide128 && !strip && (Cout % 64 == 0) && ((int64_t)tiles * (Cout / 64) * B >= 1024);
@@ -963,13 +966,13 @@
 static int conv3d_wino_entry(const float *src, int Cin, const float *a, const float *d, const void *pack, const float *out_scale,
                              const float *act_inv_scale, const float *kbias, int B, int D, int H, int W, int Cout, int relu, float *out,
                              double *out_sum, double *out_sumsq, const unsigned char *tile_active, const float *kconst, int kreach,
-                             const float *partial, void *occ_ws, size_t occ_ws_bytes, void *stream) {
+                             const float *partial, void *occ_ws, size_t occ_ws_bytes, void *stream, int src_blocked = 0, int out_blocked = 0) {
     GN_REQUIRE(pack != nullptr && Cin > 0 && Cin % SP_KS == 0 && Cout > 0 && Cout % 32 == 0, "gn_conv3d_gcr_split_wino: pack, Cin %% 16 == 0 and Cout %% 32 == 0 are required");
     GN_REQUIRE(!(kbias && act_inv_scale), "gn_conv3d_gcr_split_wino: the affine-in-weights form carries its scales in out_scale [B][Cout]");
     GN_REQUIRE(!partial || Cout % 128 != 0, "gn_conv3d_gcr_split_wino32: a polyphase partial goes with the 32-wide column-block kernel (Cout %% 128 != 0)");
     const int64_t per_sample = kbias ? (int64_t)(Cin / SP_KS) * 36 * (Cout / 32) * 2 * 1024 : 0;
     return conv3d_gcr_split_impl(src, Cin, nullptr, 0, a, d, pack, GN_SPLIT_F16X2, out_scale, act_inv_scale, B, D, H, W, Cout, relu, out, out_sum,
-                                 out_sumsq, tile_active, kconst, kreach, partial, kbias, per_sample, kbias ? Cout : 0, occ_ws, occ_ws_bytes, stream, 1);
+                                 out_sumsq, tile_active, kconst, kreach, partial, kbias, per_sample, kbias ? Cout : 0, occ_ws, occ_ws_bytes, stream, 1, src_blocked, out_blocked);
 }
 
 extern "C" int gn_conv3d_gcr_split_wino(const float *src, int Cin, const float *a, const float *d, const void *pack, const float *out_scale,
@@ -987,3 +990,11 @@
     return conv3d_wino_entry(src, Cin, a, d, pack, out_scale, act_inv_scale, kbias, B, D, H, W, Cout, relu, out, out_sum, out_sumsq, nullptr, nullptr,
                              1, partial, nullptr, 0, stream);
 }
+
+extern "C" int gn_conv3d_gcr_split_wino_blocked(const float *src, int Cin, const float *a, const float *d, const void *pack, const float *out_scale,
+                                                const float *act_inv_scale, const float *kbias, int B, int D, int H, int W, int Cout, int relu, float *out,
+                                                double *out_sum, double *out_sumsq, int src_blocked, int out_blocked, void *stream) {
+    GN_REQUIRE((src_blocked != 0) != (out_blocked != 0), "gn_conv3d_gcr_split_wino_blocked: exactly one of src_blocked / out_blocked (gn_conv3d_gcr_split_wino is the entry for neither)");
+    return conv3d_wino_entry(src, Cin, a, d, pack, out_scale, act_inv_scale, kbias, B, D, H, W, Cout, relu, out, out_sum, out_sumsq, nullptr, nullptr,
+                             1, nullptr, nullptr, 0, stream, src_blocked != 0, out_blocked != 0);
+}
diff --git a/garmentnets_amd/csrc/unet_wino.hip b/garmentnets_amd/csrc/unet_wino.hip
--- a/garmentnets_amd/csrc/unet_wino.hip
+++ b/garmentnets_amd/csrc/unet_wino.hip
@@ -307,43 +307,64 @@
             const bool interior = z0e > 0 && z0e + GN_CONV_TZ < p.D && y0e > 0 && y0e + GN_CONV_TY < p.H && x0e > 0 && x0e + GN_CONV_TX < p.W;
             const bool classes = p.kbias && !interior;
             const int mz = sp_axis_mask(gz, p.D);
-            const float *const orow = p.out + ((((int64_t)be * p.D + gz) * p.H + y0e) * p.W + x0e) * p.Cout + n0;
-            const int64_t rs2 = 2 * (int64_t)p.W * p.Cout;
-#pragma unroll
-            for (int e = 0; e < 2; ++e) {
-                const int gy = y0e + he, gx = x0e + e;
-                float kv[NT][16];
-                if (classes) {
+            const int64_t vol = (int64_t)p.D * p.H * p.W;
+            auto epilogue = [&](auto blocked_c) {
+                constexpr bool BLK = decltype(blocked_c)::value;
+                const int hi = re >> 4;
+                const float *const orow = BLK
+                    ? p.out + (int64_t)be * vol * p.Cout + (int64_t)n0 * vol + (((int64_t)gz * p.H + y0e) * p.W + x0e) * SP_KS
+                    : p.out + ((((int64_t)be * p.D + gz) * p.H + y0e) * p.W + x0e) * p.Cout + n0;
+                const int64_t rs2 = 2 * (int64_t)p.W * (BLK ? SP_KS : p.Cout);
+#pragma unroll
+                for (int e = 0; e < 2; ++e) {
+                    const int gy = y0e + he, gx = x0e + e;
+                    float kv[NT][16];
+                    if (classes) {
+#pragma unroll
+                        for (int u = 0; u < NT; ++u) {
+                            const float *kb = p.kbias + (int64_t)be * 64 * p.Cout + n0 + u * 32 + re;
+#pragma unroll
+                            for (int q = 0; q < 16; ++q)
+                                kv[u][q] = kb[(int64_t)((mz * 4 + sp_axis_mask(gy + 2 * (q >> 2), p.H)) * 4 + sp_axis_mask(gx + 2 * (q & 3), p.W)) * p.Cout];
+                        }
+                    } else {
+#pragma unroll
+                        for (int u = 0; u < NT; ++u)
+#pragma unroll
+                            for (int q = 0; q < 16; ++q) kv[u][q] = k63[u];
+                    }
 #pragma unroll
                     for (int u = 0; u < NT; ++u) {
-                        const float *kb = p.kbias + (int64_t)be * 64 * p.Cout + n0 + u * 32 + re;
-#pragma unroll
-                        for (int q = 0; q < 16; ++q)
-                            kv[u][q] = kb[(int64_t)((mz * 4 + sp_axis_mask(gy + 2 * (q >> 2), p.H)) * 4 + sp_axis_mask(gx + 2 * (q & 3), p.W)) * p.Cout];
+                        unsigned vo[4];
+#pragma unroll
+                        for (int i = 0; i < 4; ++i)
+                            vo[i] = BLK ? (unsigned)(((he * p.W + 2 * i + hi) * SP_KS + (re & 15)) * 4) : (unsigned)(((he * p.W + e + 2 * i) * p.Cout + u * 32 + re) * 4);
+#pragma unroll
+                        for (int q = 0; q < 16; ++q) {
+                            float v = __fmul_rn(tot[e][u][q], osc[u]);
+                            if (p.kbias) v = __fadd_rn(v, kv[u][q]);
+                            if (p.relu) v = gn_relu(v);
+                            const float *ob = orow + (q >> 2) * rs2;
+                            if (!BLK) {
+                                asm volatile("global_store_dword %0, %1, %2 nt" ::"v"(vo[q & 3]), "v"(v), "s"(ob) : "memory");
+                            } else if (e == 0) {
+                                tot[0][u][q] = v;
+                            } else {
+                                const float v0 = tot[0][u][q];
+                                const float got = __builtin_bit_cast(float, __builtin_amdgcn_ds_swizzle(__builtin_bit_cast(int, hi ? v0 : v), 0x401F));
+                                const float va = hi ? got : v0, vb = hi ? v : got;
+                                const float *oa = ob + (int64_t)(2 * u) * SP_KS * vol, *obk = oa + SP_KS * vol;
+                                asm volatile("global_store_dword %0, %1, %2 nt" ::"v"(vo[q & 3]), "v"(va), "s"(oa) : "memory");
+                                asm volatile("global_store_dword %0, %1, %2 nt" ::"v"(vo[q & 3]), "v"(vb), "s"(obk) : "memory");
+                            }
+                            ssum[u] += (double)v;
+                            ssq[u] += (double)v * (double)v;
+                        }
                     }
-                } else {
-#pragma unroll
-                    for (int u = 0; u < NT; ++u)
-#pragma unroll
-                        for (int q = 0; q < 16; ++q) kv[u][q] = k63[u];
-                }
-#pragma unroll
-                for (int u = 0; u < NT; ++u) {
-                    unsigned vo[4];
-#pragma unroll
-                    for (int i = 0; i < 4; ++i) vo[i] = (unsigned)(((he * p.W + e + 2 * i) * p.Cout + u * 32 + re) * 4);
-#pragma unroll
-                    for (int q = 0; q < 16; ++q) {
-                        float v = __fmul_rn(tot[e][u][q], osc[u]);
-                        if (p.kbias) v = __fadd_rn(v, kv[u][q]);
-                        if (p.relu) v = gn_relu(v);
-                        const float *ob = orow + (q >> 2) * rs2;
-                        asm volatile("global_store_dword %0, %1, %2 nt" ::"v"(vo[q & 3]), "v"(v), "s"(ob) : "memory");
-                        ssum[u] += (double)v;
-                        ssq[u] += (double)v * (double)v;
-                    }
-                }
-            }
+                }
+            };
+            if (p.out_blocked) epilogue(std::true_type{});
+            else epilogue(std::false_type{});
             if (p.osum) {
 #pragma unroll
                 for (int u = 0; u < NT; ++u) {
diff --git a/garmentnets_amd/csrc/unet_wino32.hip b/garmentnets_amd/csrc/unet_wino32.hip
--- a/garmentnets_amd/csrc/unet_wino32.hip
+++ b/garmentnets_amd/csrc/unet_wino32.hip
@@ -94,13 +94,14 @@
         int t = threadIdx.x & 255;
         asm volatile("" : "+v"(t));
         const int cq = (t & 3) * 4;
-        const unsigned vs = (unsigned)p.C0 * 4u;
+        const unsigned vw = p.src_blocked ? (unsigned)SP_KS : (unsigned)p.C0;
+        const unsigned vs = vw * 4u;
 #pragma unroll
         for (int k = 0; k < 2; ++k) {
             const int rr = stage_row(t + 256 * k), hz = rr / WL::HY, hy = rr - hz * WL::HY;
             const int gz = z0_ + hz - 1, gy = y0_ + hy - 1;
             const bool rowin = gz >= 0 && gz < p.D && gy >= 0 && gy < p.H;
-            voff1[k] = rowin ? ((unsigned)((gz * p.H + gy) * p.W + x0_) * (unsigned)p.C0 + (unsigned)cq) * 4u : (unsigned)cq * 4u;
+            voff1[k] = rowin ? ((unsigned)((gz * p.H + gy) * p.W + x0_) * vw + (unsigned)cq) * 4u : (unsigned)cq * 4u;
             const bool in0 = rowin && x0_ - 1 >= 0, in9 = rowin && x0_ + 8 < p.W;
             voff0[k] = in0 ? voff1[k] - vs : voff1[k];
             voff9[k] = in9 ? voff1[k] + 8u * vs : voff1[k];
@@ -110,7 +111,8 @@
     const float *base0 = p.src0;
     f32x4 raw[2][NIT];
     auto issue_rows = [&](int sl) {
-        const unsigned cb4 = (unsigned)sl * (SP_KS * 4u), vs = (unsigned)p.C0 * 4u;
+        const unsigned vs = p.src_blocked ? SP_KS * 4u : (unsigned)p.C0 * 4u;
+        const unsigned cb4 = (unsigned)sl * (p.src_blocked ? (unsigned)(p.D * p.H * p.W) * (SP_KS * 4u) : SP_KS * 4u);
 #pragma unroll
         for (int k = 0; k < 2; ++k) {
             if (k == 1 && !two_tasks) break;
diff --git a/garmentnets_amd/ops.py b/garmentnets_amd/ops.py
--- a/garmentnets_amd/ops.py
+++ b/garmentnets_amd/ops.py
@@ -373,16 +373,34 @@
     return SplitPack(pk.contiguous().view(torch.int16), SPLIT_F16X2, (1.0 / scale).float().contiguous())
 
 
-def conv3d_gcr_split_wino(src, a, d, pack, cout, relu=True, with_stats=False, act_inv=None, tile_active=None, kconst=None, kreach=1, partial=None):
+def conv3d_gcr_split_wino(src, a, d, pack, cout, relu=True, with_stats=False, act_inv=None, tile_active=None, kconst=None, kreach=1, partial=None,
+                          out_blocked=False):
     return _conv3d_wino("conv3d_gcr_split_wino", src, a, d, pack.tensor, pack.out_scale, act_inv, None, cout, relu, with_stats, tile_active, kconst, kreach,
-                        partial)
-
-
-def _conv3d_wino(who, src, a, d, pack, out_scale, act_inv, kbias, cout, relu, with_stats, tile_active, kconst, kreach, partial):
+                        partial, out_blocked)
+
+
+def is_blocked(x):
+    return bool(getattr(x, "_gn_blocked", False))
+
+
+def blocked_to_standard(x):
+    B, D, H, W, C = x.shape
+    return x.reshape(B, C // 16, D, H, W, 16).permute(0, 2, 3, 4, 1, 5).reshape(B, D, H, W, C).contiguous()
+
+
+def _conv3d_wino(who, src, a, d, pack, out_scale, act_inv, kbias, cout, relu, with_stats, tile_active, kconst, kreach, partial, out_blocked=False):
     B, D, H, W, C0 = src.shape
     out = torch.empty((B, D, H, W, cout), dtype=torch.float32, device=src.device)
     s, q = _stats_buffers(B, cout, src.device, with_stats)
-    if partial is not None:
+    src_blocked = is_blocked(src)
+    if src_blocked or out_blocked:
+        if tile_active is not None or partial is not None or (src_blocked and out_blocked) or (cout % 128 == 0) != bool(out_blocked):
+            raise ValueError(f"{who}: the channel-blocked form is the dense 128-wide launch's output and the dense 32-wide launch's source, nothing else")
+        _lib.call("gn_conv3d_gcr_split_wino_blocked", _p(src), C0, _p(a), _p(d), _p(pack), _p(out_scale), _p(act_inv), _p(kbias), B, D, H, W, cout,
+                  1 if relu else 0, _p(out), _p(s), _p(q), 1 if src_blocked else 0, 1 if out_blocked else 0, _stream())
+        if out_blocked:
+            out._gn_blocked = True
+    elif partial is not None:
         if tile_active is not None:
             raise ValueError(f"{who}: the occupancy-aware launch cannot take a polyphase partial")
         _lib.call("gn_conv3d_gcr_split_wino_partial", _p(src), C0, _p(a), _p(d), _p(pack), _p(out_scale), _p(act_inv), _p(kbias), B, D, H, W, cout,
@@ -502,6 +520,8 @@
 
 def conv3d_gcr_split(src0, src1, a, d, pack, cout, relu=True, with_stats=False, act_inv=None, tile_active=None, kconst=None, kreach=1,
                      partial=None):
+    if is_blocked(src0):
+        raise ValueError("conv3d_gcr_split: a channel-blocked source is read by the 32-wide Winograd launch alone")
     B, D, H, W, C0 = src0.shape
     C1 = 0 if src1 is None else src1.shape[-1]
     out = torch.empty((B, D, H, W, cout), dtype=torch.float32, device=src0.device)
@@ -542,12 +562,14 @@
     return r
 
 
-def conv3d_gcr_split_persample(src, prep, relu=True, with_stats=False, tile_active=None, kconst=None, kreach=1, partial=None):
+def conv3d_gcr_split_persample(src, prep, relu=True, with_stats=False, tile_active=None, kconst=None, kreach=1, partial=None, out_blocked=False):
     B, D, H, W, C = src.shape
     assert C == prep.cin and B == prep.stage_a.shape[0]
     if prep.wino:
         return _conv3d_wino("conv3d_gcr_split_persample", src, prep.stage_a, prep.stage_d, prep.pack, prep.out_scale, None, prep.kbias, prep.cout, relu,
-                            with_stats, tile_active, kconst, kreach, partial)
+                            with_stats, tile_active, kconst, kreach, partial, out_blocked)
+    if out_blocked or is_blocked(src):
+        raise ValueError("conv3d_gcr_split_persample: the channel-blocked form belongs to the Winograd kernels")
     out = torch.empty((B, D, H, W, prep.cout), dtype=torch.float32, device=src.device)
     s, q = _stats_buffers(B, prep.cout, src.device, with_stats)
     ows, ows_bytes = _occupancy_ws(tile_active, B, D, H, W, src.device)
@@ -572,6 +594,8 @@
 
 
 def conv3d_gcr(src0, src1, a, d, wp, cout, relu=True, with_stats=False):
+    if is_blocked(src0):
+        raise ValueError("conv3d_gcr: a channel-blocked source is read by the 32-wide Winograd launch alone")
     B, D, H, W, C0 = src0.shape
     C1 = 0 if src1 is None else src1.shape[-1]
     out = torch.empty((B, D, H, W, cout), dtype=torch.float32, device=src0.device)
diff --git a/include/garmentnets_hip.h b/include/garmentnets_hip.h
--- a/include/garmentnets_hip.h
+++ b/include/garmentnets_hip.h
@@ -129,6 +129,9 @@
 int gn_conv3d_gcr_split_wino_partial(const float *src, int Cin, const float *a, const float *d, const void *pack, const float *out_scale,
                                      const float *act_inv_scale, const float *kbias, int B, int D, int H, int W, int Cout, int relu, float *out,
                                      double *out_sum, double *out_sumsq, const float *partial, void *stream);
+int gn_conv3d_gcr_split_wino_blocked(const float *src, int Cin, const float *a, const float *d, const void *pack, const float *out_scale,
+                                     const float *act_inv_scale, const float *kbias, int B, int D, int H, int W, int Cout, int relu, float *out,
+                                     double *out_sum, double *out_sumsq, int src_blocked, int out_blocked, void *stream);
 
 int gn_upconv_partial(const float *src1, int C1, const float *a, const float *d, const void *wp, int mode, const float *out_scale,
                       const float *act_inv_scale, int B, int Dc, int Hc, int Wc, int Cout, float *partial, void *stream);
```

Result: no change. 159.0 (median of 6 runs) (+0.6%).
